# halajun/VDO_SLAM

Measured on AMD Instinct MI355X. Metric: frames/sec (per-frame hot path, KITTI-0000-shaped 1242x375) + ms/LM-iter (batch factor graph), higher is better.
Workload: dtype f64 (LM, RANSAC) / u8,i32,f32 (front-end, tracking)

## Files before the change

include/vdo_slam_hip.h:

```cpp
#ifndef VDO_SLAM_HIP_H_
#define VDO_SLAM_HIP_H_
#include <stdint.h>

#ifdef __cplusplus
extern "C" {
#endif

typedef enum vdo_status {
  VDO_OK = 0,
  VDO_ERR_INVALID = -1,
  VDO_ERR_NO_DEVICE = -2,
  VDO_ERR_OOM = -3,
  VDO_ERR_UNSUPPORTED = -4,
  VDO_ERR_INTERNAL = -5
} vdo_status;

int vdo_version(void);
const char* vdo_last_error(void);

typedef struct vdo_ctx vdo_ctx;
int vdo_ctx_create(int device, void* hip_stream, vdo_ctx** out);
int vdo_ctx_destroy(vdo_ctx* ctx);
int vdo_ctx_synchronize(vdo_ctx* ctx);
int vdo_ctx_stream(vdo_ctx* ctx, void** hip_stream_out);
// ... 31 lines not shown
  double* Hll_et;
  double* Hlp1_et;
  double* Hlp2_et;
  double* Hpp_ep;
  double chi2;
  double robust_chi2;
} vdo_ba_system;

typedef struct vdo_lm_options {
  int32_t max_iterations;
  double gain_threshold;
  int32_t verbose;
  int32_t solver;
  double pcg_tolerance;
  int32_t pcg_max_iterations;
} vdo_lm_options;

#define VDO_LM_MAX_TRACE 512
typedef struct vdo_lm_stats {
  int32_t iterations;
  int32_t total_trials;
  int32_t stop_reason;
  double initial_chi2, final_chi2, final_lambda;
  double chi2_trace[VDO_LM_MAX_TRACE];
  int32_t trials_trace[VDO_LM_MAX_TRACE];
  double ms_total, ms_linearize, ms_solve;
} vdo_lm_stats;

typedef struct vdo_ba vdo_ba;
int vdo_ba_create(vdo_ctx* ctx, const vdo_ba_graph* g, vdo_ba** out);
int vdo_ba_destroy(vdo_ba* ba);
int vdo_ba_linearize(vdo_ba* ba, int repeat, float* ms_sweep);
int vdo_ba_profile_linearize(vdo_ba* ba, int repeat, float ms[2], int64_t dims[8]);
int vdo_ba_profile_schur(vdo_ba* ba, int repeat, float* ms);
int vdo_ba_download_system(vdo_ba* ba, vdo_ba_system* out);
int vdo_ba_optimize(vdo_ba* ba, const vdo_lm_options* opt, vdo_lm_stats* stats);
int vdo_ba_get_estimates(vdo_ba* ba, double* pose_out , double* point_out );
int vdo_ba_set_estimates(vdo_ba* ba, const double* pose, const double* point);
typedef int (*vdo_allreduce_fn)(void* user, void* device_buf, int64_t count, int op);
int vdo_ba_set_allreduce(vdo_ba* ba, vdo_allreduce_fn fn, void* user, int shard_rank);
typedef struct vdo_rccl_comm vdo_rccl_comm;
int vdo_rccl_unique_id(char id_out[128]);
int vdo_rccl_comm_create(vdo_ctx* ctx, const char id[128], int n_ranks, int rank, vdo_rccl_comm** out);
int vdo_rccl_comm_destroy(vdo_rccl_comm* comm);
int vdo_rccl_comm_stats(const vdo_rccl_comm* comm, int64_t* calls, int64_t* bytes);
int vdo_rccl_allreduce(vdo_rccl_comm* comm, double* device_buf, int64_t count, int op );
int vdo_ba_set_rccl(vdo_ba* ba, vdo_rccl_comm* comm );
int vdo_ba_partition(const vdo_ba_graph* g, int world, int32_t* owner_of_point );
typedef struct vdo_ba_plan vdo_ba_plan;
int vdo_ba_plan_create(const vdo_ba_graph* g, vdo_ba_plan** out);
int vdo_ba_plan_array(const vdo_ba_plan* p, const char* name, const void** data, int64_t* count, int32_t* elem_bytes);
int vdo_ba_plan_destroy(vdo_ba_plan* p);

typedef struct vdo_flow2_problem {
  int32_t n;
  const double* obs;
  const double* flow;
  const double* depth;
  double K[4];
  double Twl[16];
  double T0[16];
  double info_flow;
  double info_prior;
  double huber_delta;
  double chi2_gate;
  int32_t max_iterations;
  int32_t ref_quirks;
} vdo_flow2_problem;

typedef struct vdo_flow2_result {
  double T[16];
  int32_t n_inliers;
  int32_t iterations, trials, stop_reason;
  double initial_chi2, final_chi2, final_lambda;
} vdo_flow2_result;

typedef struct vdo_flow2_batch vdo_flow2_batch;
int vdo_flow2_batch_create(vdo_ctx* ctx, int n_problems, const vdo_flow2_problem* probs, vdo_flow2_batch** out);
int vdo_flow2_batch_reserve(vdo_ctx* ctx, int n_problems, const int32_t* capacity, vdo_flow2_batch** out);
int vdo_flow2_batch_set(vdo_flow2_batch* batch, int k, const vdo_flow2_problem* problem);
int vdo_flow2_batch_set_T0(vdo_flow2_batch* batch, int k, const double T0[16]);
int vdo_flow2_batch_run(vdo_flow2_batch* batch);
int vdo_flow2_batch_fetch(vdo_flow2_batch* batch, vdo_flow2_result* results, double** flow_out, uint8_t** inlier_out);
int vdo_flow2_batch_destroy(vdo_flow2_batch* batch);
int vdo_flow2_optimize(vdo_ctx* ctx, const vdo_flow2_problem* p, vdo_flow2_result* result, double* flow_out, uint8_t* inlier_out);

typedef struct vdo_pose_problem {
  int32_t n;
  int32_t kind;
  const double* obs;
  const double* Xw;
  double K[4];
  double P[12];
  double T0[16];
  double huber_delta;
  double chi2_gate;
  int32_t max_iterations;
  int32_t pad;
} vdo_pose_problem;

typedef struct vdo_pose_batch vdo_pose_batch;
int vdo_pose_batch_create(vdo_ctx* ctx, int n_problems, const vdo_pose_problem* probs, vdo_pose_batch** out);
int vdo_pose_batch_run(vdo_pose_batch* batch);
int vdo_pose_batch_fetch(vdo_pose_batch* batch, vdo_flow2_result* results, uint8_t** inlier_out);
int vdo_pose_batch_destroy(vdo_pose_batch* batch);
int vdo_pose_optimize(vdo_ctx* ctx, const vdo_pose_problem* p, vdo_flow2_result* result, uint8_t* inlier_out);

typedef struct vdo_pnp_problem {
  int32_t n;
  const double* X;
  const double* uv;
  double K[4];
  int32_t max_iterations;
  double reproj_threshold;
  double confidence;
  int32_t refit;
} vdo_pnp_problem;
typedef struct vdo_pnp_result {
  double T[16];
  int32_t n_inliers;
  int32_t iterations_run;
  int32_t best_iteration;
} vdo_pnp_result;
int vdo_pnp_ransac_batch(vdo_ctx* ctx, int n_problems, const vdo_pnp_problem* probs, vdo_pnp_result* results, uint8_t** inlier_out);
int vdo_pnp_ransac_batch_overlap(vdo_ctx* ctx, int n_problems, const vdo_pnp_problem* probs, vdo_pnp_result* results, uint8_t** inlier_out,
                                 void (*host_work)(void*), void* host_arg);
int vdo_pnp_ransac_batch_gated(vdo_ctx* ctx, int n_problems, const vdo_pnp_problem* probs, vdo_pnp_result* results, uint8_t** inlier_out,
                               const int32_t* refit_above, void (*host_work)(void*), void* host_arg, void (*after_replay)(void*), void* after_arg);
int vdo_pnp_ransac(vdo_ctx* ctx, const vdo_pnp_problem* p, vdo_pnp_result* result, uint8_t* inlier_out);

typedef struct vdo_orb_params {
  int32_t n_features;
  float scale_factor;
  int32_t n_levels;
  int32_t ini_th;
  int32_t min_th;
} vdo_orb_params;

typedef struct vdo_keypoints {
  int32_t capacity, n;
  float *x, *y, *response, *angle, *size;
  int32_t* octave;
} vdo_keypoints;

typedef struct vdo_orb vdo_orb;
int vdo_orb_create(vdo_ctx* ctx, const vdo_orb_params* prm, int width, int height, vdo_orb** out);
int vdo_orb_destroy(vdo_orb* orb);
int vdo_orb_max_keypoints(const vdo_orb* orb, int* n);
int vdo_orb_last_keypoints(const vdo_orb* orb, int* n);
int vdo_orb_extract(vdo_orb* orb, const uint8_t* gray, int stride, int src_is_device, vdo_keypoints* out);
int vdo_orb_extract_begin(vdo_orb* orb, const uint8_t* gray, int stride, int src_is_device);
int vdo_orb_extract_end(vdo_orb* orb, vdo_keypoints* out);
int vdo_orb_descriptors(vdo_orb* orb, uint8_t* desc32, int capacity_rows);
int vdo_orb_extract_desc(vdo_orb* orb, const uint8_t* gray, int stride, int src_is_device, vdo_keypoints* out, uint8_t* desc32);
int vdo_orb_level_info(vdo_orb* orb, int level, int* w, int* h, int* n_features, int* n_candidates);
int vdo_orb_get_pyramid(vdo_orb* orb, int level, uint8_t* out_bordered );
int vdo_orb_get_blurred(vdo_orb* orb, int level, uint8_t* out );
int vdo_orb_get_candidates(vdo_orb* orb, int level, float* x, float* y, float* response, float* angle, int cap, int* n);
int vdo_orb_last_timing(vdo_orb* orb, double ms[2]);
int vdo_orb_tree_info(vdo_orb* orb, int level, int* on_device, int* status);
int vdo_orb_pyramid_launches(const vdo_orb* orb);


typedef struct vdo_match_set {
  int32_t n;
  const uint8_t* desc;
// ... 28 lines not shown
int vdo_frame_images_ingest_device(vdo_frame_images* f, const float* depth_dev, const float* flow_dev, const int32_t* mask_dev, float bf, float depth_map_factor,
                                   int convert_depth);
int vdo_frame_images_destroy(vdo_frame_images* f);
int vdo_frame_images_set_ctx(vdo_frame_images* f, vdo_ctx* ctx);
int vdo_frame_static_filter(vdo_frame_images* f, int n, const float* kx, const float* ky, float th_depth,
                            int32_t* keep_idx, float* corr_x, float* corr_y, float* flow_x, float* flow_y,
                            float* depth_out, int* n_out);
int vdo_frame_static_filter_sampled(vdo_frame_images* f, int n, const float* kx, const float* ky, float th_depth,
                                    int32_t* keep_idx, float* corr_x, float* corr_y, float* flow_x, float* flow_y,
                                    float* depth_out, int* n_out);
int vdo_sample_keypoints(int rows, int cols, uint64_t seed, int capacity, float* x_out, float* y_out, int* n_out);
int vdo_frame_object_sample(vdo_frame_images* f, float th_depth_obj, int step, int cap,
                            float* key_x, float* key_y, float* corr_x, float* corr_y,
                            float* flow_x, float* flow_y, float* depth_out, int32_t* label, int* n_out);
int vdo_frame_object_sample_on(vdo_ctx* on_ctx, vdo_frame_images* f, float th_depth_obj, int step, int cap,
                               float* key_x, float* key_y, float* corr_x, float* corr_y,
                               float* flow_x, float* flow_y, float* depth_out, int32_t* label, int* n_out);
int vdo_frame_filters(vdo_frame_images* f, int n, const float* kx, const float* ky, float th_depth, int sampled,
                      int32_t* keep_idx, float* s_corr_x, float* s_corr_y, float* s_flow_x, float* s_flow_y, float* s_depth, int* n_static,
                      float th_depth_obj, int step, int cap,
                      float* key_x, float* key_y, float* corr_x, float* corr_y, float* flow_x, float* flow_y, float* depth_out, int32_t* label, int* n_obj);
int vdo_frame_filters_on(vdo_ctx* on_ctx, vdo_frame_images* f, int n, const float* kx, const float* ky, float th_depth, int sampled,
                         int32_t* keep_idx, float* s_corr_x, float* s_corr_y, float* s_flow_x, float* s_flow_y, float* s_depth, int* n_static,
                         float th_depth_obj, int step, int cap,
                         float* key_x, float* key_y, float* corr_x, float* corr_y, float* flow_x, float* flow_y, float* depth_out, int32_t* label, int* n_obj);


int vdo_propagate_static(vdo_frame_images* f, int n, const float* kx, const float* ky, float* depth_out);
int vdo_propagate_object(vdo_frame_images* f, int n, const float* kx, const float* ky, float th_depth_obj,
                         float* depth_out, int32_t* label_out);
int vdo_get3d_world(vdo_ctx* ctx, int n, const float* kx, const float* ky, const float* depth,
                    const float K4[4], const float Twc[16], float* xyz_out);
int vdo_scene_flow(vdo_ctx* ctx, int n, const float* cur_x, const float* cur_y, const float* cur_d, const int32_t* cur_label, const float Tcw_cur[16],
                   const float* last_x, const float* last_y, const float* last_d, const int32_t* last_label, const float Tcw_last[16],
                   const float K4[4], float* flow3d_out, int32_t* obj_label_inout);
int vdo_renew_static(vdo_frame_images* f, int n_tm, const int32_t* tm_sta, const float* stat_x, const float* stat_y,
                     int n_orb, const float* orb_x, const float* orb_y, int max_num_sta,
                     float* key_x, float* key_y, float* corr_x, float* corr_y, float* flow_x, float* flow_y,
                     int32_t* inlier_id, float* depth_out, int* n_out);
int vdo_renew_static_world(vdo_frame_images* f, int n_tm, const int32_t* tm_sta, const float* stat_x, const float* stat_y,
                           int n_orb, const float* orb_x, const float* orb_y, int max_num_sta, const float K4[4], const float Twc[16],
                           float* key_x, float* key_y, float* corr_x, float* corr_y, float* flow_x, float* flow_y,
                           int32_t* inlier_id, float* depth_out, float* xyz_out, int* n_out);
int vdo_static_stage(vdo_frame_images* f, int n_orb, const float* orb_x, const float* orb_y, float th_depth,
                     int32_t* keep_idx, float* s_corr_x, float* s_corr_y, float* s_flow_x, float* s_flow_y, float* s_depth, int* n_static,
                     int n_tm, const int32_t* tm_sta, const float* stat_x, const float* stat_y, int max_num_sta, const float K4[4], const float Twc[16],
                     float* key_x, float* key_y, float* corr_x, float* corr_y, float* flow_x, float* flow_y,
                     int32_t* inlier_id, float* depth_out, float* xyz_out, int* n_out);
int vdo_mask_at(vdo_frame_images* f, int n, const float* cx, const float* cy, int32_t* label_out);
int vdo_mask_warp(vdo_frame_images* cur, vdo_frame_images* last, int32_t label);
int vdo_frame_images_download_mask(vdo_frame_images* f, int32_t* mask_out);
int vdo_frame_images_download_depth(vdo_frame_images* f, float* depth_out);
int vdo_frame_images_download_flow(vdo_frame_images* f, float* flow_out);


typedef struct vdo_dyn_obj_params {
  int32_t img_w, img_h;
  int32_t shrink_row, shrink_col;
  float sf_mg_thres, sf_ds_thres;
  float th_depth_obj;
  int32_t f_id;
} vdo_dyn_obj_params;
int vdo_dyn_obj_tracking(const vdo_dyn_obj_params* prm, int n, const int32_t* sem_label, int32_t* obj_label_inout,
                         const float* key_x, const float* key_y, const float* depth, const float* flow3d, const int32_t* last_sem_label,
                         int n_last_obj, const int32_t* last_sem_pos, const int32_t* last_mod_label, const uint8_t* last_obj_stat,
                         int32_t* max_id_inout, int32_t* obj_off, int32_t* obj_idx, int32_t* obj_sem, int32_t* obj_mod, int* n_obj_out);

int vdo_renew_object(vdo_frame_images* f, int n_obj, const int32_t* inl_off, const int32_t* inl_idx, const uint8_t* obj_stat,
                     const int32_t* sem_pos, const int32_t* mod_label,
                     const float* cur_x, const float* cur_y, const int32_t* cur_obj_label,
                     int n_tmp, const float* tmp_x, const float* tmp_y, const float* tmp_depth, const int32_t* tmp_label,
                     const float* tmp_flow_x, const float* tmp_flow_y, const float* tmp_corr_x, const float* tmp_corr_y,
                     int max_num_obj, int cap,
                     float* key_x, float* key_y, float* depth_out, int32_t* sem_out, float* flow_x, float* flow_y,
                     float* corr_x, float* corr_y, int32_t* dyn_inlier_id, int32_t* obj_label_out, int* n_out);
int vdo_renew_object_world(vdo_frame_images* f, int n_obj, const int32_t* inl_off, const int32_t* inl_idx, const uint8_t* obj_stat,
                           const int32_t* sem_pos, const int32_t* mod_label,
                           const float* cur_x, const float* cur_y, const int32_t* cur_obj_label,
                           int n_tmp, const float* tmp_x, const float* tmp_y, const float* tmp_depth, const int32_t* tmp_label,
                           const float* tmp_flow_x, const float* tmp_flow_y, const float* tmp_corr_x, const float* tmp_corr_y,
                           int max_num_obj, int cap, const float K4[4], const float Twc[16],
                           float* key_x, float* key_y, float* depth_out, int32_t* sem_out, float* flow_x, float* flow_y,
                           float* corr_x, float* corr_y, int32_t* dyn_inlier_id, int32_t* obj_label_out, float* xyz_out, int* n_out);

int vdo_update_mask(vdo_frame_images* cur, vdo_frame_images* last, int n, const int32_t* last_sem_label,
                    const float* last_corr_x, const float* last_corr_y, int* n_recovered);
int vdo_object_chain(vdo_frame_images* cur, vdo_frame_images* last, int n, const int32_t* last_sem_label, const float* last_corr_x, const float* last_corr_y,
                     float th_depth_obj, const float Tcw_cur[16], const float* last_x, const float* last_y, const float* last_d, const float Tcw_last[16],
                     const float K4[4], int* n_recovered, float* depth_out, int32_t* sem_out, float* flow3d_out, int32_t* obj_label_out);
int vdo_object_chain_begin(vdo_frame_images* cur, vdo_frame_images* last, int n, const int32_t* last_sem_label, const float* last_corr_x, const float* last_corr_y,
                           const float* last_x, const float* last_y, const float* last_d);
int vdo_object_chain_end(vdo_frame_images* cur, float th_depth_obj, const float Tcw_cur[16], const float Tcw_last[16], const float K4[4],
                         int* n_recovered, float* depth_out, int32_t* sem_out, float* flow3d_out, int32_t* obj_label_out);
int vdo_object_chain_prestage(vdo_ctx* ctx, int n, const int32_t* last_sem_label, const float* last_corr_x, const float* last_corr_y,
                              const float* last_x, const float* last_y, const float* last_d);

typedef struct vdo_tracks vdo_tracks;
int vdo_tracks_create(int with_object_label, vdo_tracks** out);
int vdo_tracks_destroy(vdo_tracks* t);
int vdo_tracks_add_frame(vdo_tracks* t, int n, const int32_t* asso , const int32_t* feat_label);
int vdo_tracks_size(vdo_tracks* t, int* n_tracks, int64_t* n_pairs);
int vdo_tracks_get(vdo_tracks* t, int32_t* track_off, int32_t* pair_frame, int32_t* pair_feat, int32_t* obj_id);
int vdo_tracks_get_since(vdo_tracks* t, int first_frame, int* n_tracks, int64_t* n_pairs, int32_t* track_off, int32_t* pair_frame, int32_t* pair_feat, int32_t* obj_id);

typedef struct vdo_ingest vdo_ingest;
typedef struct vdo_png_scanlines {
  const uint8_t* data;
  int64_t bytes;
  int32_t width, height, bit_depth, channels;
} vdo_png_scanlines;
enum { VDO_INGEST_MASK = 0, VDO_INGEST_FLO = 1, VDO_INGEST_DEPTH = 2, VDO_INGEST_COLOR = 3 };
int vdo_ingest_create(vdo_ctx* ctx, int width, int height, vdo_ingest** out);
int vdo_ingest_destroy(vdo_ingest* h);
int vdo_ingest_host_buffer(vdo_ingest* h, int which, int64_t bytes, void** ptr);
int vdo_ingest_device_outputs(vdo_ingest* h, uint8_t** gray, float** depth_raw, float** flow, int32_t** mask);
int vdo_ingest_frame(vdo_ingest* h, const char* mask_text, int64_t mask_bytes, const void* flo, int64_t flo_bytes, const vdo_png_scanlines* depth,
                     const vdo_png_scanlines* color, int rgb_order, uint8_t* gray, float* depth_raw, float* flow, int32_t* mask);
int vdo_ingest_last_timing(vdo_ingest* h, double ms[3]);

typedef struct vdo_stereo vdo_stereo;
typedef struct vdo_stereo_params {
  int32_t max_disparity;
  int32_t p1, p2;
  int32_t paths;
  int32_t uniqueness;
  int32_t lr_max_diff;
  int32_t subpixel;
} vdo_stereo_params;
int vdo_stereo_create(vdo_ctx* ctx, int width, int height, const vdo_stereo_params* params, vdo_stereo** out);
int vdo_stereo_destroy(vdo_stereo* h);
int vdo_stereo_compute(vdo_stereo* h, const uint8_t* left, int64_t left_stride, const uint8_t* right, int64_t right_stride, int src_is_device,
                       float* disparity256, int out_is_device, int32_t* n_valid);
int vdo_stereo_set_output_scale(vdo_stereo* h, float scale);
int vdo_stereo_get_census(vdo_stereo* h, int which, uint64_t* out);
int vdo_stereo_get_cost(vdo_stereo* h, uint8_t* out);
int vdo_stereo_get_aggregated(vdo_stereo* h, uint16_t* out);
int vdo_stereo_last_timing(vdo_stereo* h, double ms[2]);
int vdo_stereo_device_images(vdo_stereo* h, uint8_t** left, uint8_t** right, float** disparity256);
int vdo_stereo_stage_frame(vdo_stereo* h, const float* flow, const int32_t* mask, float** flow_dev, int32_t** mask_dev);

typedef struct vdo_optflow vdo_optflow;
typedef struct vdo_optflow_params {
  int32_t levels;
  int32_t radius;
  int32_t window;
  int32_t median;
  int32_t fb_max_diff;
  int32_t subpixel;
} vdo_optflow_params;
int vdo_optflow_create(vdo_ctx* ctx, int width, int height, const vdo_optflow_params* params, vdo_optflow** out);
int vdo_optflow_destroy(vdo_optflow* h);
int vdo_optflow_compute(vdo_optflow* h, const uint8_t* im0, int64_t stride0, const uint8_t* im1, int64_t stride1, int src_is_device, float* flow,
                        uint8_t* valid, int out_is_device, int32_t* n_valid);
int vdo_optflow_level_size(vdo_optflow* h, int level, int* width, int* height);
int vdo_optflow_get_pyramid(vdo_optflow* h, int which, int level, uint8_t* out);
int vdo_optflow_get_census(vdo_optflow* h, int which, int level, uint64_t* out);
int vdo_optflow_get_level_flow(vdo_optflow* h, int dir, int level, int32_t* out);
int vdo_optflow_last_timing(vdo_optflow* h, double ms[2]);
int vdo_optflow_device_images(vdo_optflow* h, uint8_t** im0, uint8_t** im1, float** flow, uint8_t** valid);
int vdo_optflow_stage_mask(vdo_optflow* h, const int32_t* mask, int32_t** mask_dev);

typedef struct vdo_labels vdo_labels;
typedef struct vdo_labels_params {
  int32_t connectivity;
  int32_t max_disp_diff;
  int32_t min_area;
// ... 207 lines not shown
```

vdo_slam_amd/csrc/capi_ctx.hip:

```cpp
#include <cstdlib>
#include <cstdarg>
#include <cstdio>

#include "../../include/vdo_slam_hip.h"
#include "ctx.hpp"

namespace {
thread_local char g_err[512] = "";
}

namespace vdo {
int set_error(int code, const char* fmt, ...) {
  va_list ap;
  va_start(ap, fmt);
  std::vsnprintf(g_err, sizeof(g_err), fmt, ap);
  va_end(ap);
  return code;
}
int ctx_bind(vdo_ctx* ctx) {
  if (!ctx) return set_error(VDO_ERR_INVALID, "null context");
  hipError_t e = hipSetDevice(ctx->device);
  if (e != hipSuccess) return set_error(VDO_ERR_NO_DEVICE, "hipSetDevice(%d): %s", ctx->device, hipGetErrorString(e));
  return VDO_OK;
}
}

extern "C" int vdo_version(void) { return 1; }
extern "C" const char* vdo_last_error(void) { return g_err; }

extern "C" int vdo_ctx_create(int device, void* hip_stream, vdo_ctx** out) {
  if (!out) return vdo::set_error(VDO_ERR_INVALID, "vdo_ctx_create: null out");
  int n = 0;
  hipError_t e = hipGetDeviceCount(&n);
  if (e != hipSuccess || n <= 0)
    return vdo::set_error(VDO_ERR_NO_DEVICE, "no HIP device available (%s); libvdo_hip has no CPU fallback",
                          e == hipSuccess ? "device count 0" : hipGetErrorString(e));
  if (device < 0 || device >= n) return vdo::set_error(VDO_ERR_INVALID, "device %d out of range [0,%d)", device, n);
  vdo_ctx* c = new vdo_ctx();
  c->device = device;
  if (hipSetDevice(device) != hipSuccess) { delete c; return vdo::set_error(VDO_ERR_NO_DEVICE, "hipSetDevice failed"); }
  if (hip_stream) { c->stream = (hipStream_t)hip_stream; c->owns_stream = false; }
  else {
    if (hipStreamCreateWithFlags(&c->stream, hipStreamNonBlocking) != hipSuccess) { delete c; return vdo::set_error(VDO_ERR_NO_DEVICE, "hipStreamCreate failed"); }
    c->owns_stream = true;
  }
  *out = c;
  return VDO_OK;
}

extern "C" int vdo_ctx_destroy(vdo_ctx* ctx) {
  if (!ctx) return VDO_OK;
  hipSetDevice(ctx->device);
  if (ctx->chain_open) {
    hipStreamSynchronize(ctx->stream);
    ctx->chain_open_free(ctx->chain_open);
  }
  if (ctx->d_arena) hipFree(ctx->d_arena);
  if (ctx->h_arena) hipHostFree(ctx->h_arena);
  if (ctx->ba_slab) hipFree(ctx->ba_slab);
  if (ctx->ba_hscal) hipHostFree(ctx->ba_hscal);
  if (ctx->ba_side) hipStreamDestroy(ctx->ba_side);
  for (hipEvent_t e : ctx->ba_ev) if (e) hipEventDestroy(e);
  if (ctx->d_stage) hipFree(ctx->d_stage);
  if (ctx->h_stage) hipHostFree(ctx->h_stage);
  if (ctx->owns_stream && ctx->stream) hipStreamDestroy(ctx->stream);
  delete ctx;
  return VDO_OK;
}

extern "C" int vdo_ctx_synchronize(vdo_ctx* ctx) {
  int rc = vdo::ctx_bind(ctx);
  if (rc != VDO_OK) return rc;
  hipError_t e = hipStreamSynchronize(ctx->stream);
  if (e != hipSuccess) return vdo::set_error(VDO_ERR_NO_DEVICE, "hipStreamSynchronize: %s", hipGetErrorString(e));
  return VDO_OK;
}

extern "C" int vdo_ctx_stream(vdo_ctx* ctx, void** hip_stream_out) {
  if (!ctx || !hip_stream_out) return vdo::set_error(VDO_ERR_INVALID, "vdo_ctx_stream: null argument");
  *hip_stream_out = (void*)ctx->stream;
  return VDO_OK;
}

extern "C" int vdo_ctx_create_cu_mask(int device, int cu_first, int cu_count, int invert, vdo_ctx** out) {
  if (!out || cu_first < 0 || cu_count <= 0) return vdo::set_error(VDO_ERR_INVALID, "vdo_ctx_create_cu_mask: bad argument");
  int n = 0;
  hipError_t e = hipGetDeviceCount(&n);
  if (e != hipSuccess || n <= 0)
    return vdo::set_error(VDO_ERR_NO_DEVICE, "no HIP device available (%s); libvdo_hip has no CPU fallback", e == hipSuccess ? "device count 0" : hipGetErrorString(e));
  if (device < 0 || device >= n) return vdo::set_error(VDO_ERR_INVALID, "device %d out of range [0,%d)", device, n);
  if (hipSetDevice(device) != hipSuccess) return vdo::set_error(VDO_ERR_NO_DEVICE, "hipSetDevice failed");
  hipDeviceProp_t prop;
  if (hipGetDeviceProperties(&prop, device) != hipSuccess) return vdo::set_error(VDO_ERR_NO_DEVICE, "hipGetDeviceProperties failed");
  const int ncu = prop.multiProcessorCount;
  if (cu_first + cu_count > ncu) return vdo::set_error(VDO_ERR_INVALID, "CU range [%d,%d) exceeds the %d CUs of the device", cu_first, cu_first + cu_count, ncu);
  const int words = (ncu + 31) / 32;
  uint32_t mask[32] = {0};
  for (int c = 0; c < ncu; ++c) {
    const bool in = c >= cu_first && c < cu_first + cu_count;
    if (in != (invert != 0)) mask[c / 32] |= 1u << (c % 32);
  }
  vdo_ctx* c = new vdo_ctx();
  c->device = device;
  if (hipExtStreamCreateWithCUMask(&c->stream, (uint32_t)words, mask) != hipSuccess) { delete c; return vdo::set_error(VDO_ERR_NO_DEVICE, "hipExtStreamCreateWithCUMask failed"); }
  c->owns_stream = true;
  *out = c;
  return VDO_OK;
}
```

vdo_slam_amd/csrc/ctx.hpp:

```cpp
#pragma once
#include <hip/hip_runtime.h>

#include <cstddef>
#include <cstdint>

struct vdo_ctx {
  int device = 0;
  hipStream_t stream = nullptr;
  bool owns_stream = false;
  char* d_arena = nullptr; size_t d_cap = 0;
  char* h_arena = nullptr; size_t h_cap = 0;
  char* h_arena_dev = nullptr;
  void* chain_open = nullptr; void (*chain_open_free)(void*) = nullptr; bool arena_held = false;
  char* d_stage = nullptr; char* h_stage = nullptr; size_t stage_cap = 0;
  int stage_n = -1, stage_L = 0;
  int32_t stage_uni[64]; int32_t stage_off[65];
  char* ba_slab = nullptr; size_t ba_slab_cap = 0, ba_slab_used = 0; bool ba_pool_busy = false;
  double* ba_hscal = nullptr; double* ba_hscal_dev = nullptr;
  hipStream_t ba_side = nullptr; hipEvent_t ba_ev[4] = {nullptr, nullptr, nullptr, nullptr};
};

namespace vdo {
int set_error(int code, const char* fmt, ...) __attribute__((format(printf, 2, 3)));
int ctx_bind(vdo_ctx* ctx);
}
```

vdo_slam_amd/csrc/flow2.hip:

```cpp
#include <algorithm>
#include <cmath>
#include <cstdlib>
#include <cstring>
#include <type_traits>
#include <vector>

#include "../../include/vdo_slam_hip.h"
#include "ctx.hpp"
#include "lm_dev.hpp"

namespace vdo {

struct Flow2Dev {
  int n, max_iterations, ref_quirks, pad;
  int64_t off;
  int64_t out_off, out_total;
  double K[4], Twl[16], T0[16];
  double info_flow, info_prior, huber_delta, huber_dsqr, chi2_gate;
};

struct Flow2Arrays {
  const double* in;
  double* om;
  double *Xw, *f0, *f1, *err, *B2a, *B2b, *hla, *hlb, *bla, *blb, *xl;
  char* out;
  int n_problems;
  struct Flow2Comm* comm;
  unsigned int tag_base;
  int max_cluster;
  int force_general;
};

constexpr int F2_CLUSTER = 8;
static_assert(F2_THREADS >= 32 * F2_CLUSTER, "cluster exchange: one thread per (workgroup, value)");
struct Flow2Slot { unsigned int lo, tag_lo, hi, tag_hi; };
struct Flow2Comm {
  Flow2Slot slot[2][F2_CLUSTER][32];
};
typedef unsigned int f2_u32x4 __attribute__((ext_vector_type(4)));
#ifndef F2_XSCOPE
#define F2_XSCOPE 2
#endif
#if F2_XSCOPE == 3
#define F2_SC "sc0 sc1"
#elif F2_XSCOPE == 2
#define F2_SC "sc1"
#else
#define F2_SC "sc0"
#endif
__device__ __forceinline__ void f2_slot_store(Flow2Slot* p, const f2_u32x4 w) { asm volatile("global_store_dwordx4 %0, %1, off " F2_SC :: "v"(p), "v"(w) : "memory"); }
__device__ __forceinline__ f2_u32x4 f2_slot_load(const Flow2Slot* p) {
  f2_u32x4 w;
  asm volatile("global_load_dwordx4 %0, %1, off " F2_SC "\n\ts_waitcnt vmcnt(0)" : "=v"(w) : "v"(p) : "memory");
  return w;
}

struct F2Pre { double B[12], b0, b1, d0, d1, d2, p2; int i; };

struct F2Lin { double B[12], h, b0, b1; };

struct F2RegStore {
  static constexpr bool kReg = true;
  const int i, tid;
  const bool active;
  double* const s_h;
  double o0 = 0, o1 = 0, m0 = 0, m1 = 0, xw[3] = {0, 0, 0};
  double fc0 = 0, fc1 = 0, ft0 = 0, ft1 = 0, xl0 = 0, xl1 = 0, er0 = 0, er1 = 0;
  F2Lin cur{}, trial{};
  double hpc = 0, hpt = 0;
  template <class F> __device__ __forceinline__ void for_each(F&& f) { if (active) f(i); }
  __device__ __forceinline__ void set_point(int, double a0, double a1, double b0, double b1, const double (&x)[3]) {
    o0 = a0; o1 = a1; m0 = b0; m1 = b1; xw[0] = x[0]; xw[1] = x[1]; xw[2] = x[2]; fc0 = b0; fc1 = b1; xl0 = 0; xl1 = 0;
  }
  __device__ __forceinline__ void point(int, double& a0, double& a1, double& b0, double& b1, double (&x)[3]) const {
    a0 = o0; a1 = o1; b0 = m0; b1 = m1; x[0] = xw[0]; x[1] = xw[1]; x[2] = xw[2];
  }
  __device__ __forceinline__ void flow_cur(int, double& f0, double& f1) const { f0 = fc0; f1 = fc1; }
  __device__ __forceinline__ void set_flow_try(int, double f0, double f1) { ft0 = f0; ft1 = f1; }
  __device__ __forceinline__ void get_xl(int, double& x0, double& x1) const { x0 = xl0; x1 = xl1; }
  __device__ __forceinline__ void set_xl(int, double x0, double x1) { xl0 = x0; xl1 = x1; }
  __device__ __forceinline__ void get_err(int, double& e0, double& e1) const { e0 = er0; e1 = er1; }
  __device__ __forceinline__ void set_err(int, double e0, double e1) { er0 = e0; er1 = e1; }
  __device__ __forceinline__ void lin_cur(int, F2Lin& L) const { L = cur; }
  template <bool TRIAL> __device__ __forceinline__ void set_lin(int, const F2Lin& L) {
    if constexpr (TRIAL) trial = L; else cur = L;
    s_h[tid] = L.h;
  }
  __device__ __forceinline__ double h_prev(int, double) const { return hpc; }
  template <bool TRIAL> __device__ __forceinline__ void after_exchange(double hb) {
    const double h = tid > 0 ? s_h[tid - 1] : hb;
    if constexpr (TRIAL) hpt = h; else hpc = h;
// ... 427 lines not shown
          if (tid < 27) s_Hc[tid] = s_red[tid];
          if (tid == 32) s_T = s_Ttry;
        } else {
          lambda *= ni; ni *= 2; built = false;
        }
        __syncthreads();
        F2_TICK(3);
        ++qmax; ++total_trials;
      } while (rho < 0 && qmax < 10);
      int result;
      if (qmax == 10 || rho == 0) result = 1;
      else {
        if ((iniChi - currentChi) * 1e3 < iniChi) nBad++; else nBad = 0;
        result = nBad >= 3 ? 1 : 0;
      }
      ok = (result == 0);
      if (!ok) stop_reason = 1;
      if (chi2_check < last_err_chi && it > 0) { ok = false; stop_reason = 2; }
      chi2_check = last_err_chi;
    }
    double cnt[1] = {0.0};
    const float gate = (float)P.chi2_gate;
    S.for_each([&](const int i) {
      double e0, e1, f0, f1;
      S.get_err(i, e0, e1);
      S.flow_cur(i, f0, f1);
      const float chi2 = (float)(e0 * (P.info_flow * e0) + e1 * (P.info_flow * e1));
      const bool outl = chi2 > gate;
      inlier_out[i] = outl ? 0 : 1;
      cnt[0] += outl ? 0.0 : 1.0;
      flow_out[2 * i] = f0;
      flow_out[2 * i + 1] = f1;
    });
    block_reduce<1>(cnt, s_scr, s_red);
    { double d_ = 0, e_ = 0; F2_CLUSTER_SUM(1, d_, e_); }
    if (tid == 0 && wg == 0) {
      se3_to_matrix(s_T, res->T);
      res->n_inliers = (int)(s_red[0] + 0.5);
      res->iterations = it; res->trials = total_trials; res->stop_reason = stop_reason;
      res->initial_chi2 = initial_chi2; res->final_chi2 = last_err_chi; res->final_lambda = lambda;
#ifdef F2_PROFILE
      for (int k = 0; k < 14; ++k) res->T[k] = (double)s_prof[k];
#endif
    }
#ifdef F2_PROFILE
    __syncthreads();
    if (tid == 0 && wg < 2) res->T[14 + wg] = (double)(__builtin_amdgcn_s_getreg((4 - 1) << 11 | 0 << 6 | 20) & 0xf) + 100.0 * blockIdx.x;
#endif
  };

  const bool REG = chunk <= F2_THREADS && !A.force_general;
  if (REG) {
    __shared__ double s_h[F2_THREADS];
    F2RegStore S{first, tid, first < c_hi, s_h};
    lm_body(S);
  } else {
    double* const om = A.om + 4 * off;
    F2MemStore S{N, first, c_lo, c_hi, om, om + 2 * (size_t)N, A.Xw + 3 * off, A.f0 + 2 * off, A.f1 + 2 * off, A.err + 2 * off, A.xl + 2 * off,
                 A.B2a + 12 * off, A.B2b + 12 * off, A.hla + off, A.hlb + off, A.bla + 2 * off, A.blb + 2 * off};
    lm_body(S);
  }
}

}

using namespace vdo;

struct vdo_flow2_batch {
  vdo_ctx* ctx = nullptr;
  int n_problems = 0;
  int64_t total = 0;
  std::vector<void*> allocs;
  Flow2Dev* d_probs = nullptr;
  Flow2Arrays A{};
  std::vector<int64_t> offs;
  std::vector<int> ns;
  char* h_pin = nullptr;
  double* h_up = nullptr;
  std::vector<Flow2Dev> hp;
  std::vector<int> caps;
  bool probs_dirty = false;
  unsigned run_seq = 0;
  const Flow2Dev* d_probs_run = nullptr;
};

extern "C" int vdo_flow2_batch_destroy(vdo_flow2_batch* b) {
  if (!b) return VDO_OK;
  if (b->ctx) { ctx_bind(b->ctx); hipStreamSynchronize(b->ctx->stream); }
  for (void* p : b->allocs) hipFree(p);
  if (b->h_pin) hipHostFree(b->h_pin);
  if (b->h_up) hipHostFree(b->h_up);
  delete b;
  return VDO_OK;
}

static void fill_descriptor(Flow2Dev& d, const vdo_flow2_problem& p) {
  d.max_iterations = p.max_iterations; d.ref_quirks = p.ref_quirks;
  std::memcpy(d.K, p.K, sizeof(d.K)); std::memcpy(d.Twl, p.Twl, sizeof(d.Twl)); std::memcpy(d.T0, p.T0, sizeof(d.T0));
  d.info_flow = p.info_flow; d.info_prior = p.info_prior; d.huber_delta = p.huber_delta;
  d.huber_dsqr = (double)(float)(p.huber_delta * p.huber_delta);
  d.chi2_gate = p.chi2_gate;
}

static void pack_planes(double* st, const vdo_flow2_problem& p) {
  const size_t n = (size_t)p.n;
  double *po = st, *pm = st + 2 * n;
  for (size_t i = 0; i < n; ++i) { po[i] = p.obs[2 * i]; po[n + i] = p.obs[2 * i + 1]; pm[i] = p.flow[2 * i]; pm[n + i] = p.flow[2 * i + 1]; }
  std::memcpy(st + 4 * n, p.depth, sizeof(double) * n);
}

extern "C" int vdo_flow2_batch_create(vdo_ctx* ctx, int n_problems, const vdo_flow2_problem* probs, vdo_flow2_batch** out) {
  if (!ctx || !probs || !out || n_problems <= 0) return set_error(VDO_ERR_INVALID, "vdo_flow2_batch_create: bad argument");
  int rc = ctx_bind(ctx);
  if (rc != VDO_OK) return rc;
  vdo_flow2_batch* b = new vdo_flow2_batch();
  b->ctx = ctx; b->n_problems = n_problems;
  std::vector<Flow2Dev> hp(n_problems);
  int64_t total = 0;
  for (int k = 0; k < n_problems; ++k) {
    const vdo_flow2_problem& p = probs[k];
    if (p.n < 0 || (p.n > 0 && (!p.obs || !p.flow || !p.depth))) { delete b; return set_error(VDO_ERR_INVALID, "flow2 problem %d: null input", k); }
    Flow2Dev& d = hp[k];
    fill_descriptor(d, p);
    d.n = p.n; d.pad = 0; d.off = total; d.out_off = total;
    b->offs.push_back(total); b->ns.push_back(p.n);
    total += p.n;
  }
  for (Flow2Dev& d : hp) d.out_total = total;
  b->total = total;
  hipStream_t s = ctx->stream;
  auto dev = [&](size_t bytes) -> void* {
    void* p = nullptr;
    if (bytes == 0) bytes = 8;
    if (hipMalloc(&p, bytes) != hipSuccess) return nullptr;
    b->allocs.push_back(p);
    return p;
  };
  const size_t T = (size_t)total, NP = (size_t)n_problems;
  std::vector<double> in(5 * T);
  for (int k = 0; k < n_problems; ++k) if (probs[k].n) pack_planes(in.data() + 5 * b->offs[k], probs[k]);
  double* d_in = (double*)dev(40 * T);
  b->d_probs = (Flow2Dev*)dev(sizeof(Flow2Dev) * NP);
  Flow2Arrays& A = b->A;
  A.in = d_in;
  A.om = (double*)dev(32 * T);
  A.Xw = (double*)dev(24 * T); A.f0 = (double*)dev(16 * T); A.f1 = (double*)dev(16 * T);
  A.err = (double*)dev(16 * T); A.B2a = (double*)dev(96 * T); A.B2b = (double*)dev(96 * T);
  A.hla = (double*)dev(8 * T); A.hlb = (double*)dev(8 * T); A.bla = (double*)dev(16 * T); A.blb = (double*)dev(16 * T);
  A.xl = (double*)dev(16 * T);
  A.n_problems = n_problems;
  A.comm = (Flow2Comm*)dev(sizeof(Flow2Comm) * NP);
  if (A.comm) hipMemsetAsync(A.comm, 0, sizeof(Flow2Comm) * NP, s);
  for (void* p : b->allocs) if (!p) { vdo_flow2_batch_destroy(b); return set_error(VDO_ERR_OOM, "hipMalloc failed"); }
  if (!d_in) { vdo_flow2_batch_destroy(b); return set_error(VDO_ERR_OOM, "hipMalloc failed"); }
  hipMemcpyAsync(d_in, in.data(), 40 * T, hipMemcpyHostToDevice, s);
  hipMemcpyAsync(b->d_probs, hp.data(), sizeof(Flow2Dev) * NP, hipMemcpyHostToDevice, s);
  if (hipHostMalloc((void**)&b->h_pin, sizeof(vdo_flow2_result) * NP + 16 * T + T + 64, hipHostMallocMapped) != hipSuccess) { b->h_pin = nullptr; vdo_flow2_batch_destroy(b); return set_error(VDO_ERR_OOM, "hipHostMalloc failed"); }
  {
    void* dp = nullptr;
    if (hipHostGetDevicePointer(&dp, b->h_pin, 0) != hipSuccess || !dp) { vdo_flow2_batch_destroy(b); return set_error(VDO_ERR_NO_DEVICE, "hipHostGetDevicePointer failed"); }
    A.out = (char*)dp;
  }
  if (hipStreamSynchronize(s) != hipSuccess) { vdo_flow2_batch_destroy(b); return set_error(VDO_ERR_NO_DEVICE, "flow2 upload failed"); }
  b->hp = hp; b->caps = b->ns;
  *out = b;
  return VDO_OK;
}

extern "C" int vdo_flow2_batch_reserve(vdo_ctx* ctx, int n_problems, const int32_t* capacity, vdo_flow2_batch** out) {
  if (!ctx || !capacity || !out || n_problems <= 0) return set_error(VDO_ERR_INVALID, "vdo_flow2_batch_reserve: bad argument");
  int64_t tot = 0;
  for (int k = 0; k < n_problems; ++k) { if (capacity[k] < 0) return set_error(VDO_ERR_INVALID, "negative capacity"); tot += capacity[k]; }
  std::vector<double> zeros(2 * (size_t)std::max<int64_t>(1, *std::max_element(capacity, capacity + n_problems)), 0.0);
  std::vector<vdo_flow2_problem> dummy(n_problems);
  for (int k = 0; k < n_problems; ++k) {
    std::memset(&dummy[k], 0, sizeof(vdo_flow2_problem));
    dummy[k].n = capacity[k]; dummy[k].obs = zeros.data(); dummy[k].flow = zeros.data(); dummy[k].depth = zeros.data();
  }
  int rc = vdo_flow2_batch_create(ctx, n_problems, dummy.data(), out);
  if (rc != VDO_OK) return rc;
  vdo_flow2_batch* b = *out;
  if (hipHostMalloc((void**)&b->h_up, sizeof(double) * 5 * (size_t)std::max<int64_t>(tot, 1) + sizeof(Flow2Dev) * (size_t)n_problems, hipHostMallocMapped) != hipSuccess) { b->h_up = nullptr; vdo_flow2_batch_destroy(b); return set_error(VDO_ERR_OOM, "hipHostMalloc failed"); }
  void* dp = nullptr;
  if (hipHostGetDevicePointer(&dp, b->h_up, 0) != hipSuccess || !dp) { vdo_flow2_batch_destroy(b); return set_error(VDO_ERR_NO_DEVICE, "hipHostGetDevicePointer failed"); }
  b->A.in = (const double*)dp;
  b->d_probs_run = (const Flow2Dev*)((const double*)dp + 5 * (size_t)std::max<int64_t>(tot, 1));
  for (int k = 0; k < n_problems; ++k) { b->hp[k].n = 0; b->ns[k] = 0; }
  std::memcpy(b->h_up + 5 * (size_t)std::max<int64_t>(tot, 1), b->hp.data(), sizeof(Flow2Dev) * (size_t)n_problems);
  if (hipStreamSynchronize(ctx->stream) != hipSuccess) { vdo_flow2_batch_destroy(b); return set_error(VDO_ERR_NO_DEVICE, "flow2 reserve failed"); }
  return VDO_OK;
}

extern "C" int vdo_flow2_batch_set(vdo_flow2_batch* b, int k, const vdo_flow2_problem* p) {
  if (!b || k < 0 || k >= b->n_problems || !b->h_up) return set_error(VDO_ERR_INVALID, "vdo_flow2_batch_set: bad argument / batch not created by vdo_flow2_batch_reserve");
  int rc = ctx_bind(b->ctx);
  if (rc != VDO_OK) return rc;
  Flow2Dev& d = b->hp[k];
  const int n = p ? p->n : 0;
  if (n < 0 || n > b->caps[k] || (n > 0 && (!p->obs || !p->flow || !p->depth))) return set_error(VDO_ERR_INVALID, "vdo_flow2_batch_set: %d points do not fit slot %d (capacity %d)", n, k, b->caps[k]);
  if (n) {
    pack_planes(b->h_up + 5 * b->offs[k], *p);
    fill_descriptor(d, *p);
  }
  d.n = n; b->ns[k] = n;
  b->probs_dirty = true;
  return VDO_OK;
}

extern "C" int vdo_flow2_batch_set_T0(vdo_flow2_batch* b, int k, const double T0[16]) {
  if (!b || k < 0 || k >= b->n_problems || !b->h_up || !T0) return set_error(VDO_ERR_INVALID, "vdo_flow2_batch_set_T0: bad argument / batch not created by vdo_flow2_batch_reserve");
  std::memcpy(b->hp[k].T0, T0, sizeof(b->hp[k].T0));
  b->probs_dirty = true;
  return VDO_OK;
}

extern "C" int vdo_flow2_batch_run(vdo_flow2_batch* b) {
  if (!b) return set_error(VDO_ERR_INVALID, "null handle");
  int rc = ctx_bind(b->ctx);
  if (rc != VDO_OK) return rc;
  if (b->probs_dirty) {
    int64_t used = 0;
    for (int k = 0; k < b->n_problems; ++k) { b->hp[k].out_off = used; used += b->hp[k].n; }
    for (int k = 0; k < b->n_problems; ++k) b->hp[k].out_total = used;
    std::memcpy(b->h_up + 5 * (size_t)std::max<int64_t>(b->total, 1), b->hp.data(), sizeof(Flow2Dev) * (size_t)b->n_problems);
    b->probs_dirty = false;
  }
  b->A.tag_base = (++b->run_seq) << 16;
  {
    int budget = 256;
    if (const char* e = std::getenv("VDO_LM_CLUSTER_BUDGET")) budget = std::max(1, std::atoi(e));
    int mc = F2_CLUSTER;
    for (; mc > 1; mc >>= 1) {
      int64_t wgs = 0;
      for (int k = 0; k < b->n_problems; ++k) if (b->ns[k] >= 3) wgs += std::min(mc, std::max(1, (b->ns[k] + F2_THREADS - 1) / F2_THREADS));
      if (wgs <= budget) break;
    }
    b->A.max_cluster = mc;
  }
  { const char* e = std::getenv("VDO_LM_GENERAL"); b->A.force_general = (e && std::atoi(e) != 0) ? 1 : 0; }
  hipLaunchKernelGGL(k_flow2_lm, dim3(((b->n_problems + 7) / 8) * 8 * F2_CLUSTER), dim3(F2_THREADS), 0, b->ctx->stream, b->d_probs_run ? b->d_probs_run : (const Flow2Dev*)b->d_probs, b->A);
  hipError_t e = hipGetLastError();
  if (e != hipSuccess) return set_error(VDO_ERR_NO_DEVICE, "k_flow2_lm launch: %s", hipGetErrorString(e));
  return VDO_OK;
}

extern "C" int vdo_flow2_batch_fetch(vdo_flow2_batch* b, vdo_flow2_result* results, double** flow_out, uint8_t** inlier_out) {
  if (!b || !results) return set_error(VDO_ERR_INVALID, "null argument");
  int rc = ctx_bind(b->ctx);
  if (rc != VDO_OK) return rc;
  const size_t NP = (size_t)b->n_problems;
  size_t used = 0;
  for (int k = 0; k < b->n_problems; ++k) used += (size_t)b->ns[k];
  hipError_t e = hipStreamSynchronize(b->ctx->stream);
  if (e != hipSuccess) return set_error(VDO_ERR_NO_DEVICE, "flow2 fetch: %s", hipGetErrorString(e));
  const vdo_flow2_result* pr = (const vdo_flow2_result*)b->h_pin;
  const double* pf = (const double*)(b->h_pin + sizeof(vdo_flow2_result) * NP);
  const uint8_t* pi = (const uint8_t*)(pf + 2 * used);
  std::memcpy(results, pr, sizeof(vdo_flow2_result) * NP);
  for (size_t k = 0; k < NP; ++k) if (pr[k].iterations < 0) return set_error(VDO_ERR_NO_DEVICE, "k_flow2_lm: the workgroup cluster of problem %d lost its barrier", (int)k);
  size_t o = 0;
  for (int k = 0; k < b->n_problems; ++k) {
    const size_t n = (size_t)b->ns[k];
    if (n && flow_out && flow_out[k]) std::memcpy(flow_out[k], pf + 2 * o, sizeof(double) * 2 * n);
    if (n && inlier_out && inlier_out[k]) std::memcpy(inlier_out[k], pi + o, n);
    o += n;
  }
  return VDO_OK;
}

extern "C" int vdo_flow2_optimize(vdo_ctx* ctx, const vdo_flow2_problem* p, vdo_flow2_result* result, double* flow_out, uint8_t* inlier_out) {
  vdo_flow2_batch* b = nullptr;
  int rc = vdo_flow2_batch_create(ctx, 1, p, &b);
  if (rc != VDO_OK) return rc;
  rc = vdo_flow2_batch_run(b);
  if (rc == VDO_OK) rc = vdo_flow2_batch_fetch(b, result, &flow_out, &inlier_out);
  vdo_flow2_batch_destroy(b);
  return rc;
}
```

vdo_slam_amd/csrc/tracking_logic.hip:

```cpp
#include <algorithm>
#include <chrono>
#include <cmath>
#include <cstring>
#include <vector>

#include "../../include/vdo_slam_hip.h"
#include "ctx.hpp"
#include "frame_images.hpp"
#include "near_flags.hpp"
#include "arena.hpp"
#include "tracking_shared.hpp"

namespace vdo {

__global__ void k_renew_obj_pred(int n, const float* __restrict__ px, const float* __restrict__ py, const int32_t* __restrict__ mask,
                                 const float* __restrict__ depth, const float* __restrict__ flow, int w, int h,
                                 int32_t* __restrict__ ok, int32_t* __restrict__ sem, float* __restrict__ dout, float* __restrict__ fx, float* __restrict__ fy) {
  const int i = blockIdx.x * blockDim.x + threadIdx.x;
  if (i >= n) return;
  const int x = (int)px[i], y = (int)py[i];
  int good = 0, sl = 0;
  float d = 0, fxe = 0, fye = 0;
  if (!(x >= w || y >= h || x <= 0 || y <= 0)) {
    const size_t o = (size_t)y * w + x;
    sl = mask[o]; d = depth[o];
    if (sl != 0 && d < 25 && d > 0) {
      fxe = flow[2 * o]; fye = flow[2 * o + 1];
      if (x + fxe < w && y + fye < h && x + fxe > 0 && y + fye > 0) good = 1;
    }
  }
  ok[i] = good; sem[i] = sl; dout[i] = d; fx[i] = fxe; fy[i] = fye;
}

__global__ void k_renew_obj_all(int n, const float* __restrict__ px, const float* __restrict__ py, const int32_t* __restrict__ mask,
                                const float* __restrict__ depth, const float* __restrict__ flow, int w, int h,
                                int32_t* __restrict__ ok, int32_t* __restrict__ sem, float* __restrict__ dout, float* __restrict__ fx, float* __restrict__ fy,
                                Cam cam, float* __restrict__ xyz_c,
                                int n_tmp, const float* __restrict__ qx, const float* __restrict__ qy, const float* __restrict__ qd, float* __restrict__ xyz_t,
                                int32_t* __restrict__ used) {
  const int i = blockIdx.x * blockDim.x + threadIdx.x;
  if (i < n) {
    const int x = (int)px[i], y = (int)py[i];
    int good = 0, sl = 0;
    float d = 0, fxe = 0, fye = 0;
    if (!(x >= w || y >= h || x <= 0 || y <= 0)) {
      const size_t o = (size_t)y * w + x;
      sl = mask[o]; d = depth[o];
      if (sl != 0 && d < 25 && d > 0) {
        fxe = flow[2 * o]; fye = flow[2 * o + 1];
        if (x + fxe < w && y + fye < h && x + fxe > 0 && y + fye > 0) good = 1;
      }
    }
    ok[i] = good; sem[i] = sl; dout[i] = d; fx[i] = fxe; fy[i] = fye;
    float o3[3];
    backproject(cam, (float)x, (float)y, d, o3);
    xyz_c[3 * i] = o3[0]; xyz_c[3 * i + 1] = o3[1]; xyz_c[3 * i + 2] = o3[2];
  }
  if (i < n_tmp) {
    used[i] = 0;
    float o3[3];
    backproject(cam, qx[i], qy[i], qd[i], o3);
    xyz_t[3 * i] = o3[0]; xyz_t[3 * i + 1] = o3[1]; xyz_t[3 * i + 2] = o3[2];
  }
}

constexpr int kVoteBins = 1024;

__global__ __launch_bounds__(256) void k_label_vote(int n, const float* __restrict__ cx, const float* __restrict__ cy,
                                                    const int32_t* __restrict__ mask, int w, int h, int32_t* __restrict__ flag) {
  __shared__ int hist[kVoteBins];
  __shared__ int s_valid, s_bad;
  for (int i = threadIdx.x; i < kVoteBins; i += 256) hist[i] = 0;
  if (threadIdx.x == 0) { s_valid = 0; s_bad = 0; }
  __syncthreads();
  for (int i = threadIdx.x; i < n; i += 256) {
    const int u = (int)cx[i], v = (int)cy[i];
    if (u < w && u > 0 && v < h && v > 0) {
      const int l = mask[(size_t)v * w + u];
      if (l < 0 || l >= kVoteBins) atomicOr(&s_bad, 1);
      else { atomicAdd(&hist[l], 1); atomicAdd(&s_valid, 1); }
    }
  }
  __syncthreads();
  __shared__ int s_cnt[256], s_lab[256];
  {
    int best = threadIdx.x * 4, cnt = hist[best];
    for (int l = best + 1; l < threadIdx.x * 4 + 4; ++l) if (hist[l] > cnt) { cnt = hist[l]; best = l; }
    s_cnt[threadIdx.x] = cnt; s_lab[threadIdx.x] = best;
  }
  __syncthreads();
  for (int step = 128; step > 0; step >>= 1) {
    if (threadIdx.x < step) {
      const int c2 = s_cnt[threadIdx.x + step], l2 = s_lab[threadIdx.x + step];
      if (c2 > s_cnt[threadIdx.x] || (c2 == s_cnt[threadIdx.x] && l2 < s_lab[threadIdx.x])) { s_cnt[threadIdx.x] = c2; s_lab[threadIdx.x] = l2; }
    }
    __syncthreads();
  }
  if (threadIdx.x == 0) {
    flag[0] = (s_valid >= 100 && s_lab[0] == 0 && !s_bad) ? 1 : 0;
    flag[1] = s_bad;
  }
}

__global__ void k_mask_warp_if(const int32_t* __restrict__ flag, const int32_t* __restrict__ mask_last, const float* __restrict__ flow_last,
                               int w, int h, int32_t lab, int32_t* __restrict__ mask_cur) {
  if (!flag[0]) return;
  const int k = blockIdx.x * blockDim.x + threadIdx.x, j = blockIdx.y;
  if (k >= w) return;
  const size_t o = (size_t)j * w + k;
  if (mask_last[o] != lab) return;
  const int fx = (int)flow_last[2 * o], fy = (int)flow_last[2 * o + 1];
  if (k + fx < w && k + fx > 0 && j + fy < h && j + fy > 0) mask_cur[(size_t)(j + fy) * w + (k + fx)] = lab;
}

struct LabelSlots { int n; int32_t lab[64]; };

__global__ __launch_bounds__(256) void k_warp_candidates(const int32_t* __restrict__ mask_last, const float* __restrict__ flow_last, int w, int h, LabelSlots T,
                                                         unsigned long long* __restrict__ cand) {
  const int k = blockIdx.x * blockDim.x + threadIdx.x, j = blockIdx.y;
  if (k >= w) return;
  const size_t o = (size_t)j * w + k;
  const int32_t lab = mask_last[o];
  int slot = -1;
  for (int s = 0; s < T.n; ++s) if (T.lab[s] == lab) slot = s;
  if (slot < 0) return;
  const int fx = (int)flow_last[2 * o], fy = (int)flow_last[2 * o + 1];
  if (k + fx < w && k + fx > 0 && j + fy < h && j + fy > 0) atomicOr(&cand[(size_t)(j + fy) * w + (k + fx)], 1ull << slot);
}

struct VoteLds { int hist[kVoteBins]; int valid, bad; int cnt[256], lab[256]; int verdict; };
__device__ __forceinline__ int vote_label(VoteLds& L, const LabelSlots& T, int s, unsigned long long rec, const int32_t* __restrict__ off, const float* __restrict__ cx,
                                          const float* __restrict__ cy, const int32_t* __restrict__ mask, const unsigned long long* __restrict__ cand, int w, int h,
                                          int32_t* __restrict__ flag) {
  for (int i = threadIdx.x; i < kVoteBins; i += 256) L.hist[i] = 0;
  if (threadIdx.x == 0) { L.valid = 0; L.bad = 0; }
  __syncthreads();
  const int lo = off[s], hi = off[s + 1];
  for (int base = lo + (int)(threadIdx.x & ~63u); base < hi; base += 4 * 256) {
    float px[4], py[4];
#pragma unroll
    for (int k = 0; k < 4; ++k) { const int i = min(base + k * 256 + (int)(threadIdx.x & 63u), hi - 1); px[k] = cx[i]; py[k] = cy[i]; }
    int ml[4]; unsigned long long mc[4]; bool in[4];
#pragma unroll
    for (int k = 0; k < 4; ++k) {
      const int i = base + k * 256 + (int)(threadIdx.x & 63u);
      const int u = (int)px[k], v = (int)py[k];
// ... 138 lines not shown
  }
  std::sort(v.begin(), v.end());
  int best = 0, cnt = -1;
  for (size_t a = 0; a < v.size();) {
    size_t b = a;
    while (b < v.size() && v[b] == v[a]) ++b;
    if ((int)(b - a) > cnt) { cnt = (int)(b - a); best = v[a]; }
    a = b;
  }
  return best;
}

}

using namespace vdo;

extern "C" int vdo_dyn_obj_tracking(const vdo_dyn_obj_params* prm, int n, const int32_t* sem_label, int32_t* obj_label_inout,
                                    const float* key_x, const float* key_y, const float* depth, const float* flow3d, const int32_t* last_sem_label,
                                    int n_last_obj, const int32_t* last_sem_pos, const int32_t* last_mod_label, const uint8_t* last_obj_stat,
                                    int32_t* max_id_inout, int32_t* obj_off, int32_t* obj_idx, int32_t* obj_sem, int32_t* obj_mod, int* n_obj_out) {
  if (!prm || !n_obj_out || !max_id_inout || n < 0 || (n > 0 && (!sem_label || !obj_label_inout || !key_x || !key_y || !depth || !flow3d || !last_sem_label)))
    return set_error(VDO_ERR_INVALID, "vdo_dyn_obj_tracking: bad argument");
  std::vector<int32_t> uni, slot;
  label_slots(n, sem_label, uni, slot);
  const int L = (int)uni.size();
  std::vector<int> cnt(L, 0);
  std::vector<float> border(L, 0.f);
  for (int i = 0; i < n; ++i) {
    if (obj_label_inout[i] == -1) continue;
    const int s = slot[i];
    ++cnt[s];
    const float u = key_x[i], v = key_y[i];
    if (v < prm->shrink_row || v > (prm->img_h - prm->shrink_row) || u < prm->shrink_col || u > (prm->img_w - prm->shrink_col)) border[s] += 1.f;
  }
  std::vector<int> state(L, 0);
  for (int s = 0; s < L; ++s) if (border[s] / (float)cnt[s] > 0.5f) state[s] = 1;
  std::vector<float> dsum(L, 0.f), slow(L, 0.f);
  for (int i = 0; i < n; ++i) {
    if (obj_label_inout[i] == -1) continue;
    const int s = slot[i];
    if (state[s] == 1) { obj_label_inout[i] = -1; continue; }
    dsum[s] = dsum[s] + depth[i];
    const float fx = flow3d[3 * i], fz = flow3d[3 * i + 2];
    if (std::sqrt(fx * fx + fz * fz) < prm->sf_mg_thres) slow[s] = slow[s] + 1.f;
  }
  for (int s = 0; s < L; ++s) {
    if (state[s]) continue;
    if (slow[s] / (float)cnt[s] > prm->sf_ds_thres) state[s] = 2;
    else if (dsum[s] / (float)cnt[s] > prm->th_depth_obj || cnt[s] < 150) state[s] = 3;
  }
  std::vector<int> acc_of(L, -1);
  int n_acc = 0;
  obj_off[0] = 0;
  for (int s = 0; s < L; ++s) if (state[s] == 0) { acc_of[s] = n_acc; obj_off[n_acc + 1] = obj_off[n_acc] + cnt[s]; obj_sem[n_acc] = uni[s]; ++n_acc; }
  std::vector<int> cur(n_acc + 1);
  for (int a = 0; a <= n_acc; ++a) cur[a] = obj_off[a];
  for (int i = 0; i < n; ++i) {
    if (obj_label_inout[i] == -1) continue;
    const int s = slot[i];
    if (state[s] == 2) obj_label_inout[i] = 0;
    else if (state[s] == 3) obj_label_inout[i] = -1;
    else if (state[s] == 0) obj_idx[cur[acc_of[s]]++] = i;
  }
  int max_id = *max_id_inout;
  if (prm->f_id == 1) max_id = 1;
  std::vector<int32_t> votes;
  for (int a = 0; a < n_acc; ++a) {
    votes.clear();
    for (int q = obj_off[a]; q < obj_off[a + 1]; ++q) votes.push_back(last_sem_label[obj_idx[q]]);
    const int new_lab = majority(votes);
    int lab = -1;
    if (max_id != 1)
      for (int k = 0; k < n_last_obj; ++k)
        if (last_sem_pos[k] == new_lab && last_obj_stat[k]) { lab = last_mod_label[k]; break; }
    if (lab == -1) { lab = max_id; max_id = max_id + 1; }
    for (int q = obj_off[a]; q < obj_off[a + 1]; ++q) obj_label_inout[obj_idx[q]] = lab;
    obj_mod[a] = lab;
  }
  *max_id_inout = max_id;
  *n_obj_out = n_acc;
  return VDO_OK;
}

extern "C" int vdo_renew_object_world(vdo_frame_images* f, int n_obj, const int32_t* inl_off, const int32_t* inl_idx, const uint8_t* obj_stat,
                                      const int32_t* sem_pos, const int32_t* mod_label,
                                      const float* cur_x, const float* cur_y, const int32_t* cur_obj_label,
                                      int n_tmp, const float* tmp_x, const float* tmp_y, const float* tmp_depth, const int32_t* tmp_label,
                                      const float* tmp_flow_x, const float* tmp_flow_y, const float* tmp_corr_x, const float* tmp_corr_y,
                                      int max_num_obj, int cap, const float K4[4], const float Twc[16],
                                      float* key_x, float* key_y, float* depth_out, int32_t* sem_out, float* flow_x, float* flow_y,
                                      float* corr_x, float* corr_y, int32_t* dyn_inlier_id, int32_t* obj_label_out, float* xyz_out, int* n_out) {
  if (!f || !n_out || n_obj < 0 || n_tmp < 0 || cap < 0 || (xyz_out && (!K4 || !Twc))) return set_error(VDO_ERR_INVALID, "vdo_renew_object: bad argument");
  int rc = ctx_bind(f->ctx);
  if (rc != VDO_OK) return rc;
  Arena S(f->ctx);
  if (!S.reserve(Arena::bytes_for(24 * ((size_t)(n_obj ? inl_off[n_obj] : 0) + (size_t)n_tmp + 64)))) return set_error(VDO_ERR_OOM, "scratch arena: allocation failed");
  static thread_local std::vector<float> cx, cy, dd, fx, fy, xyz_c, xyz_t;
  static thread_local std::vector<int32_t> cid, cobj, ok, sem, used;
  cx.clear(); cy.clear(); cid.clear(); cobj.clear();
  for (int i = 0; i < n_obj; ++i) {
    if (!obj_stat[i]) continue;
    for (int q = inl_off[i]; q < inl_off[i + 1]; ++q) { const int id = inl_idx[q]; cx.push_back(cur_x[id]); cy.push_back(cur_y[id]); cid.push_back(id); cobj.push_back(i); }
  }
  const int nc = (int)cx.size();
  ok.resize(nc); sem.resize(nc); dd.resize(nc); fx.resize(nc); fy.resize(nc);
  used.assign(n_tmp, 0);
  xyz_c.resize(xyz_out ? 3 * (size_t)nc : 0); xyz_t.resize(xyz_out ? 3 * (size_t)n_tmp : 0);
  if (nc || (n_tmp && xyz_out)) {
    float *dx = S.up(cx.data(), nc), *dy = S.up(cy.data(), nc);
    float *dqx = S.up(tmp_x, n_tmp), *dqy = S.up(tmp_y, n_tmp), *dqd = S.up(xyz_out ? tmp_depth : nullptr, xyz_out ? n_tmp : 0);
    int32_t *dok = S.up<int32_t>(nullptr, nc), *dsem = S.up<int32_t>(nullptr, nc);
    float *ddd = S.up<float>(nullptr, nc), *dfx = S.up<float>(nullptr, nc), *dfy = S.up<float>(nullptr, nc);
    int32_t* dused = S.up<int32_t>(nullptr, n_tmp);
    float *dxc = S.up<float>(nullptr, xyz_out ? 3 * (size_t)nc : 0), *dxt = S.up<float>(nullptr, xyz_out ? 3 * (size_t)n_tmp : 0);
    if (!dxt || !dxc || !dused || !dfy) return set_error(VDO_ERR_OOM, "scratch arena: allocation failed");
    hipStream_t st = S.stream();
    const Cam cam = xyz_out ? make_cam_Twc(K4, Twc) : Cam{};
    if (xyz_out) {
      const int nmax = std::max(nc, n_tmp);
      hipLaunchKernelGGL(k_renew_obj_all, dim3((nmax + 255) / 256), dim3(256), 0, st, nc, (const float*)dx, (const float*)dy, (const int32_t*)f->d_mask,
                         (const float*)f->d_depth, (const float*)f->d_flow, f->w, f->h, dok, dsem, ddd, dfx, dfy, cam, dxc,
                         n_tmp, (const float*)dqx, (const float*)dqy, (const float*)dqd, dxt, dused);
      if (nc && n_tmp) launch_near_flags_sel(st, n_tmp, dqx, dqy, nc, dx, dy, dok, 1, dused, false);
    } else if (nc) {
      hipLaunchKernelGGL(k_renew_obj_pred, dim3((nc + 255) / 256), dim3(256), 0, st, nc, (const float*)dx, (const float*)dy, (const int32_t*)f->d_mask,
                         (const float*)f->d_depth, (const float*)f->d_flow, f->w, f->h, dok, dsem, ddd, dfx, dfy);
      if (n_tmp) launch_near_flags_sel(st, n_tmp, dqx, dqy, nc, dx, dy, dok, 1, dused);
    }
    S.down(ok.data(), dok, nc); S.down(sem.data(), dsem, nc); S.down(dd.data(), ddd, nc); S.down(fx.data(), dfx, nc); S.down(fy.data(), dfy, nc);
    if (nc && n_tmp) S.down(used.data(), dused, n_tmp);
    if (xyz_out) { S.down(xyz_c.data(), dxc, 3 * (size_t)nc); S.down(xyz_t.data(), dxt, 3 * (size_t)n_tmp); }
    rc = S.finish("vdo_renew_object");
    if (rc != VDO_OK) return rc;
  }
  int m = 0;
  auto push = [&](float x, float y, float d, int sl, float flx, float fly, float crx, float cry, int inl, int ol, const float* p3) -> bool {
    if (m >= cap) return false;
    key_x[m] = x; key_y[m] = y; depth_out[m] = d; sem_out[m] = sl; flow_x[m] = flx; flow_y[m] = fly; corr_x[m] = crx; corr_y[m] = cry;
    dyn_inlier_id[m] = inl; obj_label_out[m] = ol;
    if (xyz_out) { xyz_out[3 * m] = p3[0]; xyz_out[3 * m + 1] = p3[1]; xyz_out[3 * m + 2] = p3[2]; }
    ++m;
    return true;
  };
  std::vector<int> fea_count(n_obj, -1);
  for (int i = 0; i < n_obj; ++i) if (obj_stat[i]) fea_count[i] = 0;
  for (int k = 0; k < nc; ++k) {
    if (!ok[k]) continue;
    const int x = (int)cx[k], y = (int)cy[k];
    if (!push((float)x, (float)y, dd[k], sem[k], fx[k], fy[k], x + fx[k], y + fy[k], cid[k], cur_obj_label[cid[k]], xyz_c.data() + 3 * (size_t)k)) return set_error(VDO_ERR_INVALID, "vdo_renew_object: output capacity %d too small", cap);
    ++fea_count[cobj[k]];
  }
  for (int i = 0; i < n_obj; ++i) {
    if (!obj_stat[i]) continue;
    int tot = fea_count[i];
    for (int start = 0; start < 15 && tot < max_num_obj; ++start) {
      for (int j = start; j < n_tmp; j += 15) {
        if (tmp_label[j] != sem_pos[i] || used[j]) continue;
        if (!push(tmp_x[j], tmp_y[j], tmp_depth[j], tmp_label[j], tmp_flow_x[j], tmp_flow_y[j], tmp_corr_x[j], tmp_corr_y[j], -1, mod_label[i], xyz_t.data() + 3 * (size_t)j))
          return set_error(VDO_ERR_INVALID, "vdo_renew_object: output capacity %d too small", cap);
        if (++tot >= max_num_obj) break;
      }
    }
  }
  std::vector<int32_t> uni, slot;
  label_slots(n_tmp, tmp_label, uni, slot);
  std::vector<char> known(uni.size(), 0);
  for (int i = 0; i < n_obj; ++i) {
    if (!obj_stat[i]) continue;
    auto it = std::lower_bound(uni.begin(), uni.end(), sem_pos[i]);
    if (it != uni.end() && *it == sem_pos[i]) known[it - uni.begin()] = 1;
  }
  for (size_t s = 0; s < uni.size(); ++s) {
    if (known[s]) continue;
    for (int j = 0; j < n_tmp; ++j)
      if (slot[j] == (int)s && !push(tmp_x[j], tmp_y[j], tmp_depth[j], tmp_label[j], tmp_flow_x[j], tmp_flow_y[j], tmp_corr_x[j], tmp_corr_y[j], -1, -2, xyz_t.data() + 3 * (size_t)j))
        return set_error(VDO_ERR_INVALID, "vdo_renew_object: output capacity %d too small", cap);
  }
  *n_out = m;
  return VDO_OK;
}

extern "C" int vdo_renew_object(vdo_frame_images* f, int n_obj, const int32_t* inl_off, const int32_t* inl_idx, const uint8_t* obj_stat,
                                const int32_t* sem_pos, const int32_t* mod_label,
                                const float* cur_x, const float* cur_y, const int32_t* cur_obj_label,
                                int n_tmp, const float* tmp_x, const float* tmp_y, const float* tmp_depth, const int32_t* tmp_label,
                                const float* tmp_flow_x, const float* tmp_flow_y, const float* tmp_corr_x, const float* tmp_corr_y,
                                int max_num_obj, int cap,
                                float* key_x, float* key_y, float* depth_out, int32_t* sem_out, float* flow_x, float* flow_y,
                                float* corr_x, float* corr_y, int32_t* dyn_inlier_id, int32_t* obj_label_out, int* n_out) {
  return vdo_renew_object_world(f, n_obj, inl_off, inl_idx, obj_stat, sem_pos, mod_label, cur_x, cur_y, cur_obj_label, n_tmp, tmp_x, tmp_y, tmp_depth, tmp_label,
                                tmp_flow_x, tmp_flow_y, tmp_corr_x, tmp_corr_y, max_num_obj, cap, nullptr, nullptr,
                                key_x, key_y, depth_out, sem_out, flow_x, flow_y, corr_x, corr_y, dyn_inlier_id, obj_label_out, nullptr, n_out);
}

extern "C" int vdo_update_mask(vdo_frame_images* cur, vdo_frame_images* last, int n, const int32_t* last_sem_label,
                               const float* last_corr_x, const float* last_corr_y, int* n_recovered) {
  if (!cur || !last || cur->w != last->w || cur->h != last->h || n < 0) return set_error(VDO_ERR_INVALID, "vdo_update_mask: bad argument");
  if (n_recovered) *n_recovered = 0;
  if (n == 0) return VDO_OK;
  int rc = ctx_bind(cur->ctx);
  if (rc != VDO_OK) return rc;
  Arena S(cur->ctx);
  if (!S.reserve(Arena::bytes_for(4 * (size_t)n + 512))) return set_error(VDO_ERR_OOM, "scratch arena: allocation failed");
  std::vector<int32_t> uni, slot;
  label_slots(n, last_sem_label, uni, slot);
  const int L = (int)uni.size();
  std::vector<int> off(L + 1, 0);
  for (int i = 0; i < n; ++i) off[slot[i] + 1]++;
  for (int s = 0; s < L; ++s) off[s + 1] += off[s];
  std::vector<float> gx(n), gy(n);
  {
    std::vector<int> c(off.begin(), off.end() - 1);
    for (int i = 0; i < n; ++i) { const int p = c[slot[i]]++; gx[p] = last_corr_x[i]; gy[p] = last_corr_y[i]; }
  }
  float *dx = S.up(gx.data(), n), *dy = S.up(gy.data(), n);
  std::vector<int32_t> off32(off.begin(), off.end());
  int32_t* doff = S.up(off32.data(), off32.size());
  int32_t* dflag = S.up<int32_t>(nullptr, 2 * (size_t)L);
  unsigned long long* drec = S.up<unsigned long long>(nullptr, 1);
  if (!dflag || !doff || !drec) return set_error(VDO_ERR_OOM, "hipMalloc failed");
  launch_update_mask(cur, last, uni, off, dx, dy, doff, dflag, drec, S.stream());
  std::vector<int32_t> flag(2 * (size_t)L);
  S.down(flag.data(), dflag, flag.size());
  rc = S.finish("vdo_update_mask");
  if (rc != VDO_OK) return rc;
  int rec = 0;
  for (int s = 0; s < L; ++s) {
    if (flag[2 * s + 1]) return set_error(VDO_ERR_UNSUPPORTED, "vdo_update_mask: mask label outside [0,%d)", kVoteBins);
    rec += flag[2 * s];
  }
  if (n_recovered) *n_recovered = rec;
  return VDO_OK;
}

static __global__ void k_gather_scene_flow(int n, const float* __restrict__ kx, const float* __restrict__ ky, const float* __restrict__ depth, const int32_t* __restrict__ mask,
                                           int w, int h, float th, float* __restrict__ dout, int32_t* __restrict__ lout, Cam cc,
                                           const float* __restrict__ lx, const float* __restrict__ ly, const float* __restrict__ ld, const int32_t* __restrict__ ll, Cam lc,
                                           float* __restrict__ flow3d, int32_t* __restrict__ objlab, const int32_t* __restrict__ olab_init,
                                           const int32_t* __restrict__ flag_in, int32_t* __restrict__ flag_out, int nflag) {
  const int i = blockIdx.x * blockDim.x + threadIdx.x;
  if (i < nflag) flag_out[i] = flag_in[i];
  if (i >= n) return;
  const float xf = kx[i], yf = ky[i];
  const int u = (int)xf, v = (int)yf;
  float o = 0.1f; int l = 0;
  {
    const bool inside = u < (w - 1) && u > 0 && v < (h - 1) && v > 0;
    const size_t q = inside ? (size_t)v * w + u : 0;
    const float d = depth[q];
    const int ml = mask[q];
    if (inside && d < th && d > 0) { o = d; l = ml; }
  }
  dout[i] = o; lout[i] = l;
  if (l <= 0 || ll[i] <= 0) { objlab[i] = -1; flow3d[3 * i] = 0; flow3d[3 * i + 1] = 0; flow3d[3 * i + 2] = 0; return; }
  float p[3], c[3];
  backproject(lc, lx[i], ly[i], ld[i], p);
  backproject(cc, xf, yf, o, c);
  flow3d[3 * i] = c[0] - p[0]; flow3d[3 * i + 1] = c[1] - p[1]; flow3d[3 * i + 2] = c[2] - p[2];
  objlab[i] = olab_init ? olab_init[i] : -2;
}

namespace {
struct ChainLayout { size_t gx, gy, cx, cy, lx, ly, ld, ll, off, total; };
ChainLayout chain_layout(int n) {
  auto al = [](size_t v) { return (v + 255) & ~size_t(255); };
  ChainLayout q{};
  size_t o = 0;
  const size_t b = al(4 * (size_t)n);
  q.gx = o; o += b; q.gy = o; o += b; q.cx = o; o += b; q.cy = o; o += b; q.lx = o; o += b; q.ly = o; o += b; q.ld = o; o += b; q.ll = o; o += b;
  q.off = o; o += al(4 * 65);
  q.total = o;
  return q;
}
int group_by_label(int n, const int32_t* lab, const float* px, const float* py, std::vector<int32_t>& uni, std::vector<int>& off, float* gx, float* gy) {
  static thread_local std::vector<int32_t> slot;
// ... 266 lines not shown
```

vdo_slam_amd/host/FramePipeline.cc:

```cpp
#include "FramePipeline.h"

#include "Optimizer.h"
#include "frame_math.h"

#include <algorithm>
#include <cmath>
#include <cstdio>
#include <cstdlib>
#include <cstring>
#include <thread>
#include <stdexcept>

namespace VDO_SLAM {

using namespace frame_math;

namespace {
struct SecTimer {
  double* ms; std::chrono::steady_clock::time_point t = std::chrono::steady_clock::now();
  void reset() { t = std::chrono::steady_clock::now(); }
  void tick(int slot) { const auto n = std::chrono::steady_clock::now(); ms[slot] += std::chrono::duration<double, std::milli>(n - t).count(); t = n; }
};
int await_tag(const std::atomic<int>& a, int tag) {
  for (int v;; std::this_thread::yield()) if ((v = a.load(std::memory_order_acquire)) == tag || v == -tag) return v;
}
}

class FramePipeline::Worker {
 public:
  Worker() : th_([this] { loop(); }) {}
  ~Worker() { state_.store(3, std::memory_order_release); th_.join(); }
  void run(std::function<int()> job) { job_ = std::move(job); state_.store(1, std::memory_order_release); }
  int wait() {
    if (!busy()) return 0;
    while (state_.load(std::memory_order_acquire) != 2) std::this_thread::yield();
    state_.store(0, std::memory_order_relaxed);
    return rc_;
  }
  bool busy() const { const int s = state_.load(std::memory_order_acquire); return s == 1 || s == 2; }

 private:
  void loop() {
    unsigned idle = 0;
    for (;;) {
      const int s = state_.load(std::memory_order_acquire);
      if (s == 3) return;
      if (s == 1) { rc_ = job_(); state_.store(2, std::memory_order_release); idle = 0; continue; }
      if (++idle < 200000u) continue;
      if (idle < 400000u) std::this_thread::yield(); else std::this_thread::sleep_for(std::chrono::microseconds(200));
    }
  }
  std::function<int()> job_;
  int rc_ = 0;
  std::atomic<int> state_{0};
  std::thread th_;
};

struct FramePipeline::StepState {
  FramePipeline& P;
  const uint8_t* d_gray; const float *d_depth_raw, *d_flow; const int32_t* d_mask;
  vdo_flow2_batch *cam, *obj; int n_cam_pts, n_obj_problems;
  vdo_frame_images *cur, *last;
  ObjSet& tmp;
  vdo_keypoints kp;
  const int tag;
  FrameCounts fc{};
  bool orb_pending = false, tail_via_orb = false, k10_via_orb = false, k9_via_orb = false, fin_async = false, late_upload = false, up_async = false, static_async = false,
       tail_async = false, tail_on_orb = false;
  bool orb_started = false;
  bool chain_open = false;
  int n_s = 0, n_o = 0, n_new_s = 0, n_tmp = 0, n_objects = 0;
  float Tcw[16];
  StaSet nsta; ObjSet nobj;
  std::vector<int32_t> sta_asso;
  SecTimer t;
  StepState(FramePipeline& p, const uint8_t* g, const float* d, const float* f, const int32_t* m, vdo_flow2_batch* c, vdo_flow2_batch* o, int nc, int no)
      : P(p), d_gray(g), d_depth_raw(d), d_flow(f), d_mask(m), cam(c), obj(o), n_cam_pts(nc), n_obj_problems(no), cur(p.img_[p.cur_]), last(p.img_[p.cur_ ^ 1]),
        tmp(p.tmpb_[p.cur_]), kp{(int32_t)p.kx_.size(), 0, p.kx_.data(), p.ky_.data(), p.kr_.data(), p.ka_.data(), p.ks_.data(), p.ko_.data()}, tag(p.f_id_ + 1), t{p.ms_} {}
  ~StepState() {
    if (P.worker_) P.worker_->wait();
    if (chain_open) vdo_object_chain_end(cur, 0.f, kI4, kI4, P.p_.K4, nullptr, nullptr, nullptr, nullptr, nullptr);
    for (std::atomic<int>* a : {&P.objects_done_, &P.mask_final_}) { const int v = a->load(); if (v != tag && v != -tag) a->store(-tag); }
    if (orb_started) P.worker_orb_->wait();
    if (P.worker_) P.worker_->wait();
  }
};

#define VDO_TRY(call) do { if ((call) != VDO_OK) { std::fprintf(stderr, "FramePipeline: %s\n", vdo_last_error()); return -1; } } while (0)

FramePipeline::Switches FramePipeline::ReadSwitches() {
  auto on = [](const char* name) { return std::getenv(name) != nullptr; };
  Switches w;
  w.events = on("VDO_PIPE_EVENTS"); w.trace_slow = on("VDO_PIPE_TRACE_SLOW"); w.trace_obj = on("VDO_PIPE_TRACE_OBJ"); w.trace_batch = on("VDO_BATCH_TRACE");
  w.sync_upload = on("VDO_PIPE_SYNC_UPLOAD"); w.async_upload = !on("VDO_PIPE_NO_ASYNC_UPLOAD"); w.chain_split = !on("VDO_PIPE_NO_CHAIN_SPLIT");
  w.fused_static = !on("VDO_PIPE_NO_FUSED_STATIC"); w.k9_in_static = on("VDO_PIPE_K9_IN_STATIC"); w.mm_overlap = !on("VDO_PIPE_NO_MM_OVERLAP"); w.cam_ahead = !on("VDO_PIPE_NO_CAM_AHEAD");
  return w;
}

FramePipeline::FramePipeline(vdo_ctx* ctx, vdo_ctx* ctx_lm, const PipelineParams& p, vdo_ctx* ctx_obj, vdo_ctx* ctx_worker, vdo_ctx* ctx_orb)
    : ctx_(ctx), ctx_lm_(ctx_lm), ctx_obj_(ctx_obj ? ctx_obj : ctx_lm), ctx_w_(ctx_worker ? ctx_worker : ctx), p_(p) {
  vdo_orb_params op{p.n_features, p.scale_factor, p.n_levels, p.ini_th, p.min_th};
  if (vdo_orb_create(ctx_orb ? ctx_orb : ctx, &op, p.width, p.height, &orb_) != VDO_OK) return;
  for (int k = 0; k < 2; ++k) if (vdo_frame_images_create(ctx, p.width, p.height, &img_[k]) != VDO_OK) return;
  if (vdo_tracks_create(0, &tr_sta_) != VDO_OK || vdo_tracks_create(1, &tr_dyn_) != VDO_OK) return;
  int orb_cap = 0;
  if (vdo_orb_max_keypoints(orb_, &orb_cap) != VDO_OK) return;
  const int capk = std::max(orb_cap, 3008);
  kx_.resize(capk); ky_.resize(capk); kr_.resize(capk); ka_.resize(capk); ks_.resize(capk); ko_.resize(capk);
  for (int i = 0; i < 16; ++i) Tcw_last_[i] = vel_[i] = kI4[i];
  if (p.build_lm) {
    const int32_t ccap = std::max({p.max_track_bg + 8, p.n_features + 256, orb_cap});
    if (vdo_flow2_batch_reserve(ctx_lm, 1, &ccap, &lm_cam_) != VDO_OK) return;
    std::vector<int32_t> ocap(obj_slots_, obj_cap_);
    if (vdo_flow2_batch_reserve(ctx_obj_, obj_slots_, ocap.data(), &lm_obj_) != VDO_OK) return;
  }
  store_.sta.reserve((size_t)1 << 20); store_.dyn.reserve((size_t)1 << 22);
  if (ctx_worker) worker_.reset(new Worker());
  if (ctx_worker && ctx_orb) worker_orb_.reset(new Worker());
  ctx_orb_ = ctx_orb;
  orb_split_ = ctx_orb != nullptr;
  ok_ = true;
}

FramePipeline::~FramePipeline() {
  if (worker_) { worker_->wait(); worker_.reset(); }
  if (worker_orb_) { worker_orb_->wait(); worker_orb_.reset(); }
  if (orb_) vdo_orb_destroy(orb_);
  for (int k = 0; k < 2; ++k) if (img_[k]) vdo_frame_images_destroy(img_[k]);
  if (tr_sta_) vdo_tracks_destroy(tr_sta_);
  if (tr_dyn_) vdo_tracks_destroy(tr_dyn_);
  if (lm_cam_) vdo_flow2_batch_destroy(lm_cam_);
  if (lm_obj_) vdo_flow2_batch_destroy(lm_obj_);
}

int FramePipeline::ReserveObjectSlots(int n_objects, int max_points) {
  if (n_objects <= obj_slots_ && max_points <= obj_cap_) return 0;
  const int slots = std::max(obj_slots_, (n_objects + 3) / 4 * 4), cap = std::max(obj_cap_, (max_points + 2047) / 2048 * 2048);
  std::vector<int32_t> ocap(slots, cap);
  vdo_flow2_batch* nb = nullptr;
  VDO_TRY(vdo_flow2_batch_reserve(ctx_obj_, slots, ocap.data(), &nb));
  if (lm_obj_) vdo_flow2_batch_destroy(lm_obj_);
  lm_obj_ = nb; obj_slots_ = slots; obj_cap_ = cap;
  return 0;
}

int FramePipeline::PackLm(vdo_flow2_batch* b, int slot, const std::vector<int32_t>& sub, const StaSet& S, ObjBuf& B, const double* T0, double info_prior, int max_it) {
  B.ob.clear(); B.fl.clear(); B.dp.clear();
  for (int id : sub) { B.ob.push_back(S.x[id]); B.ob.push_back(S.y[id]); B.fl.push_back(S.fx[id]); B.fl.push_back(S.fy[id]); B.dp.push_back(S.d[id]); }
  vdo_flow2_problem p;
  std::memset(&p, 0, sizeof p);
  p.n = (int)sub.size(); p.obs = B.ob.data(); p.flow = B.fl.data(); p.depth = B.dp.data();
  for (int i = 0; i < 4; ++i) p.K[i] = p_.K4[i];
  float Twl[16];
  inv_rigid(Tcw_last_, Twl);
  for (int i = 0; i < 16; ++i) { p.Twl[i] = Twl[i]; p.T0[i] = T0[i]; }
  p.info_flow = 0.1; p.info_prior = info_prior; p.huber_delta = (double)std::sqrt(0.04f); p.chi2_gate = (double)0.04f;
  p.max_iterations = max_it; p.ref_quirks = 1;
  return vdo_flow2_batch_set(b, slot, &p);
}

int FramePipeline::SeedRansac(vdo_flow2_batch* b, int slot, const double* T, float* init) {
  double T0[16];
  for (int i = 0; i < 16; ++i) T0[i] = (double)(float)T[i];
  VDO_TRY(vdo_flow2_batch_set_T0(b, slot, T0));
  if (init) for (int i = 0; i < 16; ++i) init[i] = (float)T0[i];
  return 0;
}

int FramePipeline::CameraStage() {
  SecTimer t{ms_};
  cam_run_ = nullptr; cam_n_pts_ = 0; cam_n_ransac_ = 0; cam_n_mm_ = 0;
  const int n_s = have_last_ ? (int)sta_.cx.size() : 0;
  if (have_last_ && n_s >= 4) {
    std::vector<double>&X = cam_X_, &uvd = cam_uvd_;
    X.resize(3 * (size_t)n_s); uvd.resize(2 * (size_t)n_s);
    for (int i = 0; i < n_s; ++i) {
      X[3 * i] = sta_.xyz[3 * i]; X[3 * i + 1] = sta_.xyz[3 * i + 1]; X[3 * i + 2] = sta_.xyz[3 * i + 2];
      uvd[2 * i] = sta_.cx[i]; uvd[2 * i + 1] = sta_.cy[i];
// ... 1 lines not shown
    vdo_pnp_problem pp{n_s, X.data(), uvd.data(), {p_.K4[0], p_.K4[1], p_.K4[2], p_.K4[3]}, 500, 0.4, 0.98, p_.pnp_refit};
    vdo_pnp_result pr;
    inl_ransac_cam_.assign(n_s, 0);
    float MM[16];
    int32_t mm = 0;
    bool use_ransac = false;
    int rc_set = VDO_OK;
    std::function<void()> count_mm = [&] {
      mul44(vel_, Tcw_last_, MM);
      inl_mm_cam_.resize(n_s);
      mm = count_mm_inliers(MM, p_.K4, n_s, nullptr, sta_.xyz.data(), sta_.cx.data(), sta_.cy.data(), inl_mm_cam_.data());
    };
    std::function<void()> pack_lm = [&] {
      if (!lm_cam_) return;
      use_ransac = pr.n_inliers > mm;
      const std::vector<uint8_t>& flag = use_ransac ? inl_ransac_cam_ : inl_mm_cam_;
      double T0[16];
      for (int i = 0; i < 16; ++i) T0[i] = (double)MM[i];
      cam_subset_.clear();
      for (int i = 0; i < n_s; ++i) if (flag[i]) cam_subset_.push_back(i);
      rc_set = PackLm(lm_cam_, 0, cam_subset_, sta_, cam_buf_, T0, 0.3, 100);
      cam_run_ = lm_cam_; cam_n_pts_ = (int)cam_subset_.size();
      for (int i = 0; i < 16; ++i) Tcw_init_[i] = (float)T0[i];
    };
    auto call = [](void* f) { (*static_cast<std::function<void()>*>(f))(); };
    uint8_t* rip = inl_ransac_cam_.data();
    VDO_TRY(vdo_pnp_ransac_batch_gated(ctx_, 1, &pp, &pr, &rip, &mm, +call, &count_mm, +call, &pack_lm));
    cam_n_ransac_ = pr.n_inliers; cam_n_mm_ = mm;
    if (rc_set != VDO_OK) { std::fprintf(stderr, "FramePipeline: %s\n", vdo_last_error()); return -1; }
    if (lm_cam_ && use_ransac && SeedRansac(lm_cam_, 0, pr.T, Tcw_init_) != 0) return -1;
  } else if (lm_cam_) {
    for (int i = 0; i < 16; ++i) Tcw_init_[i] = Tcw_last_[i];
    VDO_TRY(vdo_flow2_batch_set(lm_cam_, 0, nullptr));
    if (have_last_) { cam_run_ = lm_cam_; cam_n_pts_ = 0; }
  }
  if (cam_run_) VDO_TRY(vdo_flow2_batch_run(cam_run_));
  t.tick(kSecK1K11RansacCam);
  return 0;
}

int FramePipeline::Step(const uint8_t* d_gray, const float* d_depth_raw, const float* d_flow, const int32_t* d_mask,
                        vdo_flow2_batch* cam, vdo_flow2_batch* obj, int n_cam_pts, int n_obj_problems, FrameCounts* out) {
  if (!ok_) return -1;
  const auto t_step0 = std::chrono::steady_clock::now();
  ev_on_ = sw_.events; ev_t0_ = t_step0;
  double ms0[kSecCount];
  for (int i = 0; i < kSecCount; ++i) ms0[i] = ms_[i];
  orb_ready_.store(0, std::memory_order_relaxed); objects_done_.store(0, std::memory_order_relaxed); mask_final_.store(0, std::memory_order_relaxed);
  StepState s(*this, d_gray, d_depth_raw, d_flow, d_mask, cam, obj, n_cam_pts, n_obj_problems);
  if (StartOrb(s) != 0) return -1;
  if (pending_ && worker_) {
    vdo_frame_images_set_ctx(ho_.img, ctx_w_);
    worker_->run([this, sp = &s] { return FinishObjects(&sp->fc, true); });
    s.fin_async = true;
  }
  if (IngestImages(s) != 0) return -1;
  if (CameraAndLateUpload(s) != 0) return -1;
  if (sw_.chain_split && have_last_ && !pending_ && BeginChain(s) != 0) return -1;
  mark(kEvChainBegun);
  if (ConsumeCamera(s) != 0) return -1;
  if (JoinLastObjects(s) != 0) return -1;
  if (EndChain(s) != 0) return -1;
  if (s.tail_async && !s.tail_on_orb && worker_->wait() != 0) return -1;
  if (have_last_ && worker_) {
    vdo_frame_images_set_ctx(s.cur, ctx_w_);
    worker_->run([this, sp = &s] { return StaticStage(*sp); });
    s.static_async = true;
  }
  if (!have_last_) { if (InitFirstFrame(s) != 0) return -1; }
  else {
    if (ObjectProblems(s) != 0) return -1;
    if (s.obj) VDO_TRY(vdo_flow2_batch_run(s.obj));
    mark(kEvObjLmLaunched);
    if (s.static_async) {
      const int rc = worker_->wait();
      vdo_frame_images_set_ctx(s.cur, ctx_);
      if (rc != 0) return -1;
    } else if (StaticStage(s) != 0) return -1;
    if ((s.tail_on_orb || s.k10_via_orb) && worker_orb_->wait() != 0) return -1;
    if (s.k10_via_orb) s.fc.n_object_samples = s.n_tmp;
    if (s.k9_via_orb) s.fc.n_static_new = s.n_new_s;
    mark(kEvStaticJoined);
    s.t.reset();
    ho_.n_objects = s.n_objects; ho_.obj_run = s.obj; ho_.n_obj_problems = s.n_obj_problems; ho_.n_tmp = s.n_tmp; ho_.img = s.cur; ho_.f_id = f_id_; ho_.tmp_idx = cur_;
    std::memcpy(ho_.Tcw, s.Tcw, sizeof s.Tcw);
    pending_ = true;
  }
  s.t.tick(kSecTracklets);
  CommitFrame(s);
  if (sw_.cam_ahead && lm_cam_ && !cam_ahead_) {
    if (CameraStage() != 0) return -1;
    cam_ahead_ = true;
    mark(kEvCamStageDone);
  }
  if (host_inputs_ && depth_inout_ && !depth_metric_ && pending_ && !p_.defer_objects) {
    VDO_TRY(vdo_frame_images_download_depth(img_[cur_ ^ 1], depth_inout_));
    depth_on_host_ = true;
  }
  if (pending_ && !p_.defer_objects) { if (FinishObjects(&s.fc) != 0) return -1; mark(kEvObjDone); }
  mark(kEvStepEnd);
  if (sw_.trace_slow) {
    const double tot = std::chrono::duration<double, std::milli>(std::chrono::steady_clock::now() - t_step0).count();
    if (tot > 2.5) {
      std::fprintf(stderr, "[slow step f=%d] %.2f ms:", f_id_ - 1, tot);
      for (int i = 0; i < kSecCount; ++i) std::fprintf(stderr, " [%d] %.2f", i, ms_[i] - ms0[i]);
      std::fprintf(stderr, "\n");
    }
  }
  if (out) *out = s.fc;
  return 0;
}

int FramePipeline::StartOrb(StepState& s) {
  s.orb_pending = worker_orb_ && !p_.use_sample_feature;
  s.tail_via_orb = s.orb_pending && pending_ && worker_;
  s.k10_via_orb = s.orb_pending && have_last_ && worker_;
  s.k9_via_orb = s.k10_via_orb && !sw_.k9_in_static;
  if (s.orb_pending) {
    worker_orb_->run([this, sp = &s] { return OrbJob(*sp); });
    s.orb_started = true;
  } else if (orb_split_ && !p_.use_sample_feature) VDO_TRY(vdo_orb_extract_begin(orb_, s.d_gray, p_.width, host_inputs_ ? 0 : 1));
  return 0;
}

int FramePipeline::OrbJob(StepState& s) {
  SecTimer t{ms_};
  int rc = vdo_orb_extract(orb_, s.d_gray, p_.width, host_inputs_ ? 0 : 1, &s.kp) == VDO_OK ? 0 : -1;
  t.tick(kSecOrb);
  if (rc != 0) std::fprintf(stderr, "FramePipeline: %s\n", vdo_last_error());
  mark(kEvOrbDone);
  orb_ready_.store(rc == 0 ? s.tag : -s.tag, std::memory_order_release);
  if (s.tail_via_orb && await_tag(objects_done_, s.tag) == s.tag) {
    const int rc2 = FinishObjectsTail(&s.fc);
    tail_done_.store(true, std::memory_order_release);
    if (rc2 != 0) rc = rc2;
  }
  if (s.k10_via_orb && await_tag(mask_final_, s.tag) == s.tag && (s.k9_via_orb && rc == 0 ? FiltersOnOrb(s) : SampleObjectsOnOrb(s)) != 0) rc = -1;
  return rc;
}

void FramePipeline::SizeFilterOutputs(int n) {
  keep_.resize(std::max(n, 1));
  for (auto* v : {&flt_cx_, &flt_cy_, &flt_fx_, &flt_fy_, &flt_d_}) v->resize(std::max(n, 1));
}
void FramePipeline::SizeSampleOutputs(ObjSet& tmp) {
  const int cap_s = SampleCap();
  tmp.x.resize(cap_s); tmp.y.resize(cap_s); tmp.cx.resize(cap_s); tmp.cy.resize(cap_s); tmp.fx.resize(cap_s); tmp.fy.resize(cap_s); tmp.d.resize(cap_s); tmp.sem.resize(cap_s);
}

int FramePipeline::SampleObjectsOnOrb(StepState& s) {
  SecTimer t{ms_};
  ObjSet& tmp = s.tmp;
  SizeSampleOutputs(tmp);
  VDO_TRY(vdo_frame_object_sample_on(ctx_orb_, s.cur, p_.th_depth_obj, 4, SampleCap(), tmp.x.data(), tmp.y.data(), tmp.cx.data(), tmp.cy.data(), tmp.fx.data(), tmp.fy.data(), tmp.d.data(),
                                     tmp.sem.data(), &s.n_tmp));
  t.tick(kSecK10OnOrb);
  return 0;
}

int FramePipeline::FiltersOnOrb(StepState& s) {
  SecTimer t{ms_};
  ObjSet& tmp = s.tmp;
  SizeFilterOutputs(s.kp.n);
  SizeSampleOutputs(tmp);
  VDO_TRY(vdo_frame_filters_on(ctx_orb_, s.cur, s.kp.n, kx_.data(), ky_.data(), p_.th_depth_bg, 0, keep_.data(), flt_cx_.data(), flt_cy_.data(), flt_fx_.data(), flt_fy_.data(),
                               flt_d_.data(), &s.n_new_s, p_.th_depth_obj, 4, SampleCap(), tmp.x.data(), tmp.y.data(), tmp.cx.data(), tmp.cy.data(), tmp.fx.data(), tmp.fy.data(),
// ... 260 lines not shown
}

int FramePipeline::ObjectProblems(StepState& s) {
  const int n_o = s.n_o;
  vdo_dyn_obj_params dp{p_.width, p_.height, 25, 50, p_.sf_mg_thres, p_.sf_ds_thres, p_.th_depth_obj, f_id_};
  std::vector<int32_t>&off = ho_.off, &idx = ho_.idx, &osem = ho_.osem, &omod = ho_.omod;
  off.assign(n_o + 2, 0); idx.resize(std::max(n_o, 1)); osem.resize(n_o + 1); omod.resize(n_o + 1);
  int n_objects = 0;
  VDO_TRY(vdo_dyn_obj_tracking(&dp, n_o, obj_sem_.data(), ho_.olab.data(), obj_.cx.data(), obj_.cy.data(), obj_depth_.data(), flow3d_.data(), obj_.sem.data(),
                               (int)last_sem_pos_.size(), last_sem_pos_.data(), last_mod_label_.data(), last_obj_stat_.data(), &max_id_,
                               off.data(), idx.data(), osem.data(), omod.data(), &n_objects));
  s.fc.n_objects = s.n_objects = n_objects;
  s.t.tick(kSecK13DynObj); mark(kEvDynObj);
  if (n_objects > 0) {
    std::vector<double>&X = obj_X_, &uvd = obj_uvd_;
    X.resize(3 * (size_t)off[n_objects] + 3); uvd.resize(2 * (size_t)off[n_objects] + 2);
    std::vector<vdo_pnp_problem> pp(n_objects);
    std::vector<vdo_pnp_result> pr(n_objects);
    for (int a = 0; a < n_objects; ++a) {
      for (int q = off[a]; q < off[a + 1]; ++q) {
        const int id = idx[q];
        X[3 * q] = obj_.xyz[3 * id]; X[3 * q + 1] = obj_.xyz[3 * id + 1]; X[3 * q + 2] = obj_.xyz[3 * id + 2];
        uvd[2 * q] = obj_.cx[id]; uvd[2 * q + 1] = obj_.cy[id];
      }
      pp[a] = vdo_pnp_problem{off[a + 1] - off[a], X.data() + 3 * (size_t)off[a], uvd.data() + 2 * (size_t)off[a], {p_.K4[0], p_.K4[1], p_.K4[2], p_.K4[3]}, 500, 0.4, 0.98, p_.pnp_refit};
    }
    inl_ransac_.assign((size_t)off[n_objects] + 1, 0);
    std::vector<uint8_t*> rip(n_objects);
    for (int a = 0; a < n_objects; ++a) rip[a] = inl_ransac_.data() + off[a];
    inl_mm_.assign((size_t)off[n_objects] + 1, 0);
    ho_.use_mm.assign(n_objects, 0);
    obj_mm_.resize(16 * (size_t)n_objects);
    std::vector<int> mm_cnt(n_objects, -1);
    int rc_pack = 0;
    std::function<void()> count_mm = [&] { CountObjectMotionModels(s.Tcw, n_objects, mm_cnt.data()); };
    std::function<void()> pack_lms = [&] { rc_pack = PackObjectLms(n_objects, pr.data(), mm_cnt.data()); };
    auto call = [](void* f) { (*static_cast<std::function<void()>*>(f))(); };
    if (sw_.mm_overlap) VDO_TRY(vdo_pnp_ransac_batch_gated(ctx_, n_objects, pp.data(), pr.data(), rip.data(), mm_cnt.data(), +call, &count_mm, +call, &pack_lms));
    else { VDO_TRY(vdo_pnp_ransac_batch(ctx_, n_objects, pp.data(), pr.data(), rip.data())); count_mm(); pack_lms(); }
    if (rc_pack != 0) { if (rc_pack == -2) std::fprintf(stderr, "FramePipeline: %s\n", vdo_last_error()); return -1; }
    for (int a = 0; a < n_objects; ++a) s.fc.n_ransac_obj += pr[a].n_inliers;
    for (int a = 0; a < n_objects; ++a) {
      if (mm_cnt[a] < 0) continue;
      s.fc.n_mm_inliers_obj += mm_cnt[a];
      if (ho_.use_mm[a]) ++s.fc.n_motion_model_obj;
    }
    if (lm_obj_) {
      for (int a = 0; a < n_objects; ++a) if (ho_.stat[a] && !ho_.use_mm[a] && SeedRansac(lm_obj_, a, pr[a].T, nullptr) != 0) return -1;
      s.obj = lm_obj_; s.n_obj_problems = obj_slots_;
    }
  } else if (lm_obj_) {
    for (int a = 0; a < obj_slots_; ++a) VDO_TRY(vdo_flow2_batch_set(lm_obj_, a, nullptr));
    s.obj = nullptr;
  }
  s.t.tick(kSecRansacObj); mark(kEvObjLmBuilt);
  return 0;
}

void FramePipeline::CommitFrame(StepState& s) {
  StaSet& nsta = s.nsta; ObjSet& nobj = s.nobj;
  const float* Tcw = s.Tcw;
  s.fc.n_static_tracked = (int)nsta.x.size();
  int64_t np = 0;
  vdo_tracks_size(tr_sta_, &s.fc.n_static_tracks, &np);
  if (keep_graph_) {
    store_.sta.append(nsta.x.size(), nsta.x.data(), nsta.y.data(), nsta.d.data(), nsta.xyz.data());
    float Twc_m[16];
    inv_rigid(Tcw, Twc_m);
    store_.add_camera(Twc_m);
    if (!have_last_) store_.dyn.append(nobj.x.size(), nobj.x.data(), nobj.y.data(), nobj.d.data(), nobj.xyz.data());
  }
  sta_ = std::move(nsta);
  if (!have_last_) { s.fc.n_object_tracked = (int)nobj.x.size(); obj_ = std::move(nobj); vdo_tracks_size(tr_dyn_, &s.fc.n_dynamic_tracks, &np); }
  float Twl[16];
  inv_rigid(Tcw_last_, Twl);
  mul44(Tcw, Twl, vel_);
  inv_rigid(vel_, cam_motion_);
  std::memcpy(Tcw_last_, Tcw, sizeof s.Tcw);
  std::memcpy(Tcw_out_, Tcw, sizeof s.Tcw);
  cur_ ^= 1; have_last_ = true; ++f_id_;
  gate_last_ = gate_cur_;
}

int FramePipeline::FinishObjects(FrameCounts* fcp, bool defer_tail) {
  if (!pending_) return 0;
  FrameCounts dummy{};
  FrameCounts& fc = fcp ? *fcp : dummy;
  SecTimer t{ms_};
  const int n_objects = ho_.n_objects, n_tmp = ho_.n_tmp, n_obj_problems = ho_.n_obj_problems;
  vdo_flow2_batch* obj = ho_.obj_run;
  const float* Tcw = ho_.Tcw;
  std::vector<int32_t>&olab = ho_.olab, &off = ho_.off, &idx = ho_.idx, &osem = ho_.osem, &omod = ho_.omod;
  ObjSet& tmp = tmpb_[ho_.tmp_idx];
  ObjSet nobj;
  std::vector<int32_t> dyn_asso;
  float Twc[16];
  inv_rigid(Tcw, Twc);
  motions_.clear();
  {
    cur_ox_ = obj_.cx; cur_oy_ = obj_.cy;
    std::vector<uint8_t> stat(std::max(n_objects, 1), 1);
    std::vector<int32_t>*p_off = &off, *p_idx = &idx;
    if (obj && obj == lm_obj_) {
      const int NS = n_obj_problems;
      std::vector<vdo_flow2_result>& rs = lm_rs_;
      std::vector<std::vector<double>>& fo = lm_fo_; std::vector<std::vector<uint8_t>>& io = lm_io_;
      std::vector<double*>& fop = lm_fop_; std::vector<uint8_t*>& iop = lm_iop_;
      rs.resize(NS); fop.resize(NS); iop.resize(NS);
      if ((int)fo.size() < NS) { fo.resize(NS); io.resize(NS); }
      for (int a = 0; a < NS; ++a) {
        const size_t na = (a < n_objects && ho_.stat[a]) ? ho_.subsets[a].size() : 0;
        fo[a].resize(2 * na + 2); io[a].resize(na + 1);
        fop[a] = fo[a].data(); iop[a] = io[a].data();
      }
      VDO_TRY(vdo_flow2_batch_fetch(obj, rs.data(), fop.data(), iop.data()));
      mark(kEvObjLmFetched);
      if (sw_.trace_obj) {
        std::fprintf(stderr, "[obj lm f=%d]", ho_.f_id);
        for (int a = 0; a < n_objects; ++a)
          if (ho_.stat[a]) std::fprintf(stderr, " sem %d n %zu its %d trials %d inl %d |", osem[a], ho_.subsets[a].size(), rs[a].iterations, rs[a].trials, rs[a].n_inliers);
        std::fprintf(stderr, "\n");
      }
      inl_off_.assign(1, 0); inl_idx_.clear();
      for (int a = 0; a < n_objects; ++a) {
        stat[a] = ho_.stat[a];
        if (stat[a]) {
          const std::vector<int32_t>& sub = ho_.subsets[a];
          for (size_t j = 0; j < sub.size(); ++j) {
            if (!io[a][j]) { olab[sub[j]] = -1; continue; }
            inl_idx_.push_back(sub[j]);
            cur_ox_[sub[j]] = key_plus_flow(obj_.x[sub[j]], fo[a][2 * j]); cur_oy_[sub[j]] = key_plus_flow(obj_.y[sub[j]], fo[a][2 * j + 1]);
          }
          ObjectMotion om; om.mod_label = omod[a]; om.sem_label = osem[a]; om.n_inliers = rs[a].n_inliers;
          float TH[16];
          for (int i = 0; i < 16; ++i) TH[i] = (float)rs[a].T[i];
          mul44(Twc, TH, om.H);
          motions_.push_back(om);
        } else {
          for (int q = off[a]; q < off[a + 1]; ++q) inl_idx_.push_back(idx[q]);
        }
        inl_off_.push_back((int32_t)inl_idx_.size());
      }
      if (inl_idx_.empty()) inl_idx_.push_back(0);
      p_off = &inl_off_; p_idx = &inl_idx_;
    } else if (obj) {
      std::vector<vdo_flow2_result> rs(std::max(n_obj_problems, 1));
      VDO_TRY(vdo_flow2_batch_fetch(obj, rs.data(), nullptr, nullptr));
    }
    t.tick(kSecWaitObjLm);
    const int cap_o = (*p_off)[n_objects] + n_tmp + 8;
    nobj.x.resize(cap_o); nobj.y.resize(cap_o); nobj.cx.resize(cap_o); nobj.cy.resize(cap_o); nobj.fx.resize(cap_o); nobj.fy.resize(cap_o); nobj.d.resize(cap_o);
    nobj.sem.resize(cap_o); nobj.label.resize(cap_o); dyn_asso.resize(cap_o);
    int mo = 0;
    nobj.xyz.resize(3 * (size_t)std::max(cap_o, 1));
    VDO_TRY(vdo_renew_object_world(ho_.img, n_objects, p_off->data(), p_idx->data(), stat.data(), osem.data(), omod.data(), cur_ox_.data(), cur_oy_.data(), olab.data(),
                                   n_tmp, tmp.x.data(), tmp.y.data(), tmp.d.data(), tmp.sem.data(), tmp.fx.data(), tmp.fy.data(), tmp.cx.data(), tmp.cy.data(),
                                   p_.max_track_obj, cap_o, p_.K4, Twc, nobj.x.data(), nobj.y.data(), nobj.d.data(), nobj.sem.data(), nobj.fx.data(), nobj.fy.data(),
                                   nobj.cx.data(), nobj.cy.data(), dyn_asso.data(), nobj.label.data(), nobj.xyz.data(), &mo));
    for (auto* v : {&nobj.x, &nobj.y, &nobj.cx, &nobj.cy, &nobj.fx, &nobj.fy, &nobj.d}) v->resize(mo);
    nobj.sem.resize(mo); nobj.label.resize(mo); dyn_asso.resize(mo);
    nobj.xyz.resize(3 * (size_t)std::max(mo, 1));
    t.tick(kSecRenewObject); mark(kEvObjRenewed);
    last_sem_pos_.assign(osem.begin(), osem.begin() + n_objects);
    last_mod_label_.assign(omod.begin(), omod.begin() + n_objects);
    last_obj_stat_.assign(stat.begin(), stat.begin() + n_objects);
    last_obj_mod_.assign(16 * (size_t)n_objects, 0.f);
    for (int a = 0, m = 0; a < n_objects; ++a) {
      float* Hd = last_obj_mod_.data() + 16 * (size_t)a;
      if (obj && obj == lm_obj_ && stat[a] && m < (int)motions_.size()) std::memcpy(Hd, motions_[m++].H, 64);
      else std::memcpy(Hd, kI4, 64);
    }
  }
  fc.n_object_tracked = (int)nobj.x.size();
  obj_ = std::move(nobj);
  if (!p_.defer_objects && !obj_.cx.empty())
    VDO_TRY(vdo_object_chain_prestage(ctx_, (int)obj_.cx.size(), obj_.sem.data(), obj_.cx.data(), obj_.cy.data(), obj_.x.data(), obj_.y.data(), obj_.d.data()));
  ho_.dyn_asso_tail = std::move(dyn_asso);
  ho_.tail_has_lm = obj && obj == lm_obj_;
  pending_ = false; tail_pending_ = true;
  return defer_tail ? 0 : FinishObjectsTail(&fc);
}

int FramePipeline::FinishObjectsTail(FrameCounts* fcp) {
  if (!tail_pending_) return 0;
  FrameCounts dummy{};
  FrameCounts& fc = fcp ? *fcp : dummy;
  SecTimer t{ms_};
  const ObjSet& nobj = obj_;
  const int f_id_obj = ho_.f_id;
  VDO_TRY(vdo_tracks_add_frame(tr_dyn_, (int)nobj.x.size(), ho_.dyn_asso_tail.data(), nobj.label.data()));
  t.tick(kSecTracklets);
  int64_t np = 0;
  vdo_tracks_size(tr_dyn_, &fc.n_dynamic_tracks, &np);
  if (keep_graph_) {
    store_.dyn.append(nobj.x.size(), nobj.x.data(), nobj.y.data(), nobj.d.data(), nobj.xyz.data());
    std::vector<float> mots(cam_motion_, cam_motion_ + 16); std::vector<int32_t> labs(1, 0);
    if (ho_.tail_has_lm)
      for (const ObjectMotion& om : motions_) { mots.insert(mots.end(), om.H, om.H + 16); labs.push_back(om.mod_label); }
    store_.add_motions((int)labs.size(), mots.data(), labs.data());
    const int Wn = p_.window_size, Ov = p_.overlap_size;
    if (Wn > 0 && Wn > Ov && (f_id_obj - Ov + 1) % (Wn - Ov) == 0 && f_id_obj >= Wn - 1 && store_.sta.frames() == f_id_obj + 1) {
      const auto t_gt0 = std::chrono::steady_clock::now();
      if (GetTracks(&tl_sta_, nullptr, f_id_obj + 1 - Wn) != 0) return -1;
      if (sw_.trace_batch) std::fprintf(stderr, "[partial batch] static tracklets flattened in %.2f ms (%zu tracks, %zu entries)\n", std::chrono::duration<double, std::milli>(std::chrono::steady_clock::now() - t_gt0).count(), tl_sta_.off.size() - 1, tl_sta_.frame.size());
      try { Optimizer::PartialBatchOptimization(store_, tl_sta_, p_.K4, Wn); }
      catch (const std::exception& e) { std::fprintf(stderr, "FramePipeline: %s\n", e.what()); return -1; }
      ++n_partial_batches_;
    }
  }
  tail_pending_ = false;
  return 0;
}

int FramePipeline::StepHost(const uint8_t* gray, const float* depth, const float* flow, const int32_t* mask, bool depth_is_metric, FrameCounts* out, float* depth_inout) {
  host_inputs_ = true; depth_metric_ = depth_is_metric; depth_inout_ = depth_inout;
  const int rc = Step(gray, depth, flow, mask, nullptr, nullptr, 0, 0, out);
  host_inputs_ = false; depth_metric_ = false; depth_inout_ = nullptr;
  return rc;
}

int FramePipeline::StepDevice(const uint8_t* d_gray, const float* d_depth, const float* d_flow, const int32_t* d_mask, bool depth_is_metric, FrameCounts* out) {
  depth_metric_ = depth_is_metric;
  const int rc = Step(d_gray, d_depth, d_flow, d_mask, nullptr, nullptr, 0, 0, out);
  depth_metric_ = false;
  return rc;
}

int FramePipeline::DownloadMask(int32_t* mask_out) {
  VDO_TRY(vdo_frame_images_download_mask(img_[cur_ ^ 1], mask_out));
  return 0;
}

int FramePipeline::DownloadDepth(float* depth_out) {
  VDO_TRY(vdo_frame_images_download_depth(img_[cur_ ^ 1], depth_out));
  return 0;
}

int FramePipeline::FinalizeMap() {
  if (!map_) return -1;
  if (pending_ && FinishObjects(nullptr) != 0) return -1;
  return SyncMap();
// ... 149 lines not shown
```

vdo_slam_amd/host/FramePipeline.h:

```cpp
#pragma once
#include <chrono>
#include <cstdint>
#include <functional>
#include <memory>
#include <atomic>
#include <vector>

#include "../../include/vdo_slam_hip.h"
#include "GraphStore.h"
#include "Map.h"

namespace VDO_SLAM {

struct PipelineParams {
  int width, height;
  float K4[4];
  float bf, depth_map_factor;
  float th_depth_bg, th_depth_obj;
  int max_track_bg, max_track_obj;
  float sf_mg_thres, sf_ds_thres;
  int n_features, n_levels, ini_th, min_th; float scale_factor;
  int build_lm;
  int defer_objects;
  int use_sample_feature;
  int sample_seed;
  int pnp_refit;
  int window_size, overlap_size;
};

struct FrameCounts { int n_orb, n_static_new, n_object_samples, n_static_tracked, n_object_tracked, n_objects, n_recovered_masks, n_static_tracks, n_dynamic_tracks,
                         n_ransac_cam, n_motion_model_cam, n_ransac_obj, n_cam_inliers, cam_lm_iterations,
                         n_mm_inliers_obj,
                         n_motion_model_obj; };

class FramePipeline {
 public:
  FramePipeline(vdo_ctx* ctx, vdo_ctx* ctx_lm, const PipelineParams& p, vdo_ctx* ctx_obj = nullptr, vdo_ctx* ctx_worker = nullptr, vdo_ctx* ctx_orb = nullptr);
  ~FramePipeline();
  int Step(const uint8_t* d_gray, const float* d_depth_raw, const float* d_flow, const int32_t* d_mask,
           vdo_flow2_batch* cam, vdo_flow2_batch* obj, int n_cam_pts, int n_obj_problems, FrameCounts* out);
  int StepHost(const uint8_t* gray, const float* depth, const float* flow, const int32_t* mask, bool depth_is_metric, FrameCounts* out, float* depth_inout = nullptr);
  int StepDevice(const uint8_t* d_gray, const float* d_depth, const float* d_flow, const int32_t* d_mask, bool depth_is_metric, FrameCounts* out);
  bool DepthConvertedOnHost() const { return depth_on_host_; }
  void SetObjectGate(const int* labels, int n) { gate_on_ = true; gate_cur_.assign(labels, labels + n); }
  int DownloadMask(int32_t* mask_out);
  int DownloadDepth(float* depth_out);
  vdo_frame_images* LastImages() { return img_[cur_ ^ 1]; }
  void KeepGraph() { keep_graph_ = true; }
  void AttachMap(Map* m) { map_ = m; keep_graph_ = true; }
  int SyncMap();
  int FinalizeMap();
  int FullBatchOptimization();
  const GraphStore& store() const { return store_; }
  int n_partial_batches_ = 0;
  int Flush(FrameCounts* fc = nullptr) { return FinishObjects(fc); }
  int GetTracks(TrackList* sta, TrackList* dyn, int first_frame = -1);
  bool ok() const { return ok_; }
  void SetDeferObjects(bool on) { p_.defer_objects = on ? 1 : 0; }
  const PipelineParams& params() const { return p_; }
  struct ObjectMotion { int mod_label, sem_label, n_inliers; float H[16]; };
  std::vector<ObjectMotion> motions_;
  float Tcw_out_[16] = {1, 0, 0, 0, 0, 1, 0, 0, 0, 0, 1, 0, 0, 0, 0, 1};
  enum { kSecK1K11RansacCam = 0, kSecOrb, kSecK9K10, kSecWaitCamLm, kSecK13DynObj, kSecRenewStatic, kSecWaitObjLm, kSecRenewObject, kSecTracklets, kSecRansacObj,
         kSecK15K11Objects, kSecK10OnOrb, kSecCount };
  double ms_[kSecCount] = {0};
  enum { kEvInputs = 0, kEvCamFetched, kEvObjChain, kEvDynObj, kEvObjLmBuilt, kEvObjLmLaunched, kEvOrbDevice, kEvOrbDone, kEvFilters, kEvStaticDone,
         kEvStaticJoined, kEvCamStageDone, kEvObjLmFetched, kEvObjRenewed, kEvObjDone, kEvStepEnd, kEvChainBegun, kEvCount };
  double ev_ms_[kEvCount] = {0}; long ev_n_[kEvCount] = {0};
  bool ev_on_ = false;
  std::chrono::steady_clock::time_point ev_t0_;
  void mark(int k) { if (ev_on_) { ev_ms_[k] += std::chrono::duration<double, std::milli>(std::chrono::steady_clock::now() - ev_t0_).count(); ++ev_n_[k]; } }

  struct StaSet { std::vector<float> x, y, cx, cy, fx, fy, d, xyz; };
  struct ObjSet : StaSet { std::vector<int32_t> sem, label; };
  const StaSet& StaticSet() const { return sta_; }
  const ObjSet& ObjectSet() const { return obj_; }
  const ObjSet& ObjectSamples() const { return tmpb_[ho_.tmp_idx]; }
  int NumObjectSamples() const { return ho_.n_tmp; }
  const std::vector<int32_t>& ObjSemPosition() const { return last_sem_pos_; }
  const std::vector<int32_t>& ObjModLabel() const { return last_mod_label_; }
  const std::vector<uint8_t>& ObjStat() const { return last_obj_stat_; }
  const std::vector<float>& ObjMod() const { return last_obj_mod_; }
  int MaxId() const { return max_id_; }

 private:
  struct Switches { bool events, trace_slow, trace_obj, trace_batch, sync_upload, async_upload, chain_split, fused_static, k9_in_static, mm_overlap, cam_ahead; };
  static Switches ReadSwitches();
  const Switches sw_ = ReadSwitches();
  struct StepState;
  int StartOrb(StepState& s), OrbJob(StepState& s), SampleObjectsOnOrb(StepState& s), FiltersOnOrb(StepState& s), JoinOrb(StepState& s);
  int IngestImages(StepState& s);
  int CameraAndLateUpload(StepState& s);
  int BeginChain(StepState& s);
  int ConsumeCamera(StepState& s);
  int JoinLastObjects(StepState& s);
  int EndChain(StepState& s);
  int FrameFilters(StepState& s), StaticStage(StepState& s);
  int InitFirstFrame(StepState& s);
  int ObjectProblems(StepState& s);
  void CommitFrame(StepState& s);
  int CameraStage();
  int FinishObjects(FrameCounts* fc, bool defer_tail = false);
  int FinishObjectsTail(FrameCounts* fc);
  void CountObjectMotionModels(const float* Tcw, int n_objects, int* cnt);
  int PackObjectLms(int n_objects, const vdo_pnp_result* pr, const int* mm_cnt);
  int SampleCap() const { return ((p_.width + 3) / 4) * ((p_.height + 3) / 4); }
  void SizeFilterOutputs(int n);
  void SizeSampleOutputs(ObjSet& tmp);
  bool tail_pending_ = false;
  GraphStore store_;
  TrackList tl_sta_, tl_dyn_;
  bool keep_graph_ = false;
  bool host_inputs_ = false, depth_metric_ = false, gate_on_ = false;
  float* depth_inout_ = nullptr;
  bool depth_on_host_ = false;
  std::vector<int> gate_cur_, gate_last_;
  Map* map_ = nullptr;
  float cam_motion_[16];
  class Worker;
  std::unique_ptr<Worker> worker_;
  std::unique_ptr<Worker> worker_orb_;
  std::atomic<bool> tail_done_{true};
  bool orb_split_ = false;
  vdo_ctx *ctx_, *ctx_lm_, *ctx_obj_, *ctx_w_, *ctx_orb_ = nullptr;
  struct ObjHandOver {
    std::vector<int32_t> olab, off, idx, osem, omod;
    int n_objects = 0, n_obj_problems = 0, n_tmp = 0, f_id = 0, tmp_idx = 0;
    vdo_flow2_batch* obj_run = nullptr; vdo_frame_images* img = nullptr; float Tcw[16];
    std::vector<std::vector<int32_t>> subsets;
    std::vector<uint8_t> stat, use_mm;
    std::vector<int32_t> dyn_asso_tail; bool tail_has_lm = false;
  } ho_;
  bool pending_ = false;
  PipelineParams p_;
  vdo_orb* orb_ = nullptr;
  vdo_frame_images* img_[2] = {nullptr, nullptr};
  vdo_tracks *tr_sta_ = nullptr, *tr_dyn_ = nullptr;
  int cur_ = 0, f_id_ = 0;
  bool ok_ = false, have_last_ = false;
  int32_t max_id_ = 1;
  StaSet sta_;
  ObjSet tmpb_[2];
  std::atomic<int> orb_ready_{0};
  std::atomic<int> objects_done_{0};
  std::atomic<int> mask_final_{0};
  ObjSet obj_;
  std::vector<int32_t> last_sem_pos_, last_mod_label_; std::vector<uint8_t> last_obj_stat_;
  std::vector<float> last_obj_mod_;
  float Tcw_last_[16], vel_[16];
  std::vector<float> kx_, ky_, kr_, ka_, ks_; std::vector<int32_t> ko_;
  std::vector<float> stat_depth_, obj_depth_, flow3d_;
  std::vector<int32_t> obj_sem_, keep_, tm_;
  std::vector<float> flt_cx_, flt_cy_, flt_fx_, flt_fy_, flt_d_;
  std::vector<float> cur_sx_, cur_sy_, cur_ox_, cur_oy_, src_x_, src_y_;
  std::vector<double> flow_out_; std::vector<uint8_t> inl_out_, inl_ransac_;
  std::vector<double> obj_X_, obj_uvd_, cam_X_, cam_uvd_;
  int obj_slots_ = 8, obj_cap_ = 6000;
  int ReserveObjectSlots(int n_objects, int max_points);
  struct ObjBuf { std::vector<double> ob, fl, dp; };
  int PackLm(vdo_flow2_batch* b, int slot, const std::vector<int32_t>& sub, const StaSet& S, ObjBuf& B, const double* T0, double info_prior, int max_it);
  int SeedRansac(vdo_flow2_batch* b, int slot, const double* T, float* init);
  vdo_flow2_batch *lm_cam_ = nullptr, *lm_obj_ = nullptr;
  std::vector<int32_t> cam_subset_, inl_off_, inl_idx_;
  std::vector<vdo_flow2_result> lm_rs_; std::vector<std::vector<double>> lm_fo_; std::vector<std::vector<uint8_t>> lm_io_;
  std::vector<double*> lm_fop_; std::vector<uint8_t*> lm_iop_;
  std::vector<uint8_t> inl_mm_;
  std::vector<float> obj_mm_;
  std::vector<ObjBuf> obj_buf_; ObjBuf cam_buf_;
  float Tcw_init_[16];
  bool cam_ahead_ = false;
  vdo_flow2_batch* cam_run_ = nullptr;
  int cam_n_pts_ = 0, cam_n_ransac_ = 0, cam_n_mm_ = 0;
  std::vector<uint8_t> inl_ransac_cam_, inl_mm_cam_;
};

}
```

vdo_slam_amd/tracking.py:

```python
import ctypes as C

import numpy as np

from . import _capi as K


def _f(a): return np.ascontiguousarray(a, dtype=np.float32)
def _i(a): return np.ascontiguousarray(a, dtype=np.int32)
def _fp(a): return a.ctypes.data_as(K.c_float_p)
def _ip(a): return a.ctypes.data_as(K.c_int32_p)


_bound = False


def _lib():
    global _bound
    L = K.lib()
    if not _bound:
        fp, ip, vp = K.c_float_p, K.c_int32_p, C.c_void_p
        L.vdo_propagate_static.argtypes = [vp, C.c_int, fp, fp, fp]
        L.vdo_propagate_object.argtypes = [vp, C.c_int, fp, fp, C.c_float, fp, ip]
        L.vdo_get3d_world.argtypes = [vp, C.c_int, fp, fp, fp, fp, fp, fp]
        L.vdo_scene_flow.argtypes = [vp, C.c_int, fp, fp, fp, ip, fp, fp, fp, fp, ip, fp, fp, fp, ip]
# ... 86 lines not shown
    if world is not None:
        out["xyz"] = xyz[:n]
    return k9, out


def mask_at(images, cx, cy):
    cx, cy = _f(cx), _f(cy)
    out = np.zeros(cx.size, np.int32)
    K.check(_lib().vdo_mask_at(images._h, cx.size, _fp(cx), _fp(cy), _ip(out)))
    return out


def mask_warp(cur_images, last_images, label):
    K.check(_lib().vdo_mask_warp(cur_images._h, last_images._h, int(label)))


class DynObjParamsC(C.Structure):
    _fields_ = [("img_w", C.c_int32), ("img_h", C.c_int32), ("shrink_row", C.c_int32), ("shrink_col", C.c_int32),
                ("sf_mg_thres", C.c_float), ("sf_ds_thres", C.c_float), ("th_depth_obj", C.c_float), ("f_id", C.c_int32)]


def _u8p(a): return a.ctypes.data_as(K.c_uint8_p)


def dyn_obj_tracking(prm: DynObjParamsC, sem_label, obj_label, key_x, key_y, depth, flow3d, last_sem_label,
                     last_sem_pos, last_mod_label, last_obj_stat, max_id):
    sem, ol = _i(sem_label), _i(obj_label).copy()
    kx, ky, d, fl, ls = _f(key_x), _f(key_y), _f(depth), _f(flow3d), _i(last_sem_label)
    lsp, lml = _i(last_sem_pos), _i(last_mod_label)
    lst = np.ascontiguousarray(last_obj_stat, dtype=np.uint8)
    n = sem.size
    nl = max(1, np.unique(sem).size)
    off = np.zeros(nl + 1, np.int32); idx = np.zeros(max(n, 1), np.int32); osem = np.zeros(nl, np.int32); omod = np.zeros(nl, np.int32)
    mid = C.c_int32(max_id); nobj = C.c_int()
    L = K.lib()
    L.vdo_dyn_obj_tracking.argtypes = [C.POINTER(DynObjParamsC), C.c_int, K.c_int32_p, K.c_int32_p, K.c_float_p, K.c_float_p, K.c_float_p, K.c_float_p,
                                       K.c_int32_p, C.c_int, K.c_int32_p, K.c_int32_p, K.c_uint8_p, C.POINTER(C.c_int32),
                                       K.c_int32_p, K.c_int32_p, K.c_int32_p, K.c_int32_p, C.POINTER(C.c_int)]
    K.check(L.vdo_dyn_obj_tracking(C.byref(prm), n, _ip(sem), _ip(ol), _fp(kx), _fp(ky), _fp(d), _fp(fl), _ip(ls), lsp.size, _ip(lsp), _ip(lml), _u8p(lst),
                                   C.byref(mid), _ip(off), _ip(idx), _ip(osem), _ip(omod), C.byref(nobj)))
    k = nobj.value
    return dict(obj_label=ol, objects=[idx[off[a]:off[a + 1]].copy() for a in range(k)], sem=osem[:k].copy(), mod=omod[:k].copy(), max_id=mid.value)


def renew_object(images, inl_sets, obj_stat, sem_pos, mod_label, cur_x, cur_y, cur_obj_label, tmp, max_num_obj, cap=None, world=None):
    off = np.zeros(len(inl_sets) + 1, np.int32)
    off[1:] = np.cumsum([len(s) for s in inl_sets])
    idx = _i(np.concatenate([np.asarray(s, np.int32) for s in inl_sets])) if len(inl_sets) and off[-1] else np.zeros(1, np.int32)
    st = np.ascontiguousarray(obj_stat, dtype=np.uint8)
    sp, ml = _i(sem_pos), _i(mod_label)
    cx, cy, col = _f(cur_x), _f(cur_y), _i(cur_obj_label)
    t = {k: (_i(v) if k == "label" else _f(v)) for k, v in tmp.items()}
    n_tmp = t["x"].size
    cap = cap or (int(off[-1]) + n_tmp + 8)
    f = [np.zeros(cap, np.float32) for _ in range(7)]
    sem = np.zeros(cap, np.int32); inl = np.zeros(cap, np.int32); ol = np.zeros(cap, np.int32)
    n = C.c_int()
    L = K.lib()
    fp, ip = K.c_float_p, K.c_int32_p
    L.vdo_renew_object.argtypes = [C.c_void_p, C.c_int, ip, ip, K.c_uint8_p, ip, ip, fp, fp, ip, C.c_int, fp, fp, fp, ip, fp, fp, fp, fp, C.c_int, C.c_int,
                                   fp, fp, fp, ip, fp, fp, fp, fp, ip, ip, C.POINTER(C.c_int)]
    if world is None:
        K.check(L.vdo_renew_object(images._h, len(inl_sets), _ip(off), _ip(idx), _u8p(st), _ip(sp), _ip(ml), _fp(cx), _fp(cy), _ip(col),
                                   n_tmp, _fp(t["x"]), _fp(t["y"]), _fp(t["depth"]), _ip(t["label"]), _fp(t["flow_x"]), _fp(t["flow_y"]), _fp(t["corr_x"]), _fp(t["corr_y"]),
                                   max_num_obj, cap, _fp(f[0]), _fp(f[1]), _fp(f[2]), _ip(sem), _fp(f[3]), _fp(f[4]), _fp(f[5]), _fp(f[6]), _ip(inl), _ip(ol), C.byref(n)))
    else:
        K4, Twc = _f(world[0]), _f(world[1])
        xyz = np.zeros((cap, 3), np.float32)
        L.vdo_renew_object_world.argtypes = [C.c_void_p, C.c_int, ip, ip, K.c_uint8_p, ip, ip, fp, fp, ip, C.c_int, fp, fp, fp, ip, fp, fp, fp, fp, C.c_int, C.c_int, fp, fp,
                                             fp, fp, fp, ip, fp, fp, fp, fp, ip, ip, fp, C.POINTER(C.c_int)]
        K.check(L.vdo_renew_object_world(images._h, len(inl_sets), _ip(off), _ip(idx), _u8p(st), _ip(sp), _ip(ml), _fp(cx), _fp(cy), _ip(col),
                                         n_tmp, _fp(t["x"]), _fp(t["y"]), _fp(t["depth"]), _ip(t["label"]), _fp(t["flow_x"]), _fp(t["flow_y"]), _fp(t["corr_x"]), _fp(t["corr_y"]),
                                         max_num_obj, cap, _fp(K4), _fp(Twc), _fp(f[0]), _fp(f[1]), _fp(f[2]), _ip(sem), _fp(f[3]), _fp(f[4]), _fp(f[5]), _fp(f[6]), _ip(inl), _ip(ol),
                                         _fp(xyz), C.byref(n)))
    m = n.value
    names = ("key_x", "key_y", "depth", "flow_x", "flow_y", "corr_x", "corr_y")
    out = {k: a[:m] for k, a in zip(names, f)}
    out.update(sem=sem[:m], inlier_id=inl[:m], obj_label=ol[:m])
    if world is not None:
        out["xyz"] = xyz[:m]
    return out


def update_mask(cur_images, last_images, last_sem_label, last_corr_x, last_corr_y):
    sl, cx, cy = _i(last_sem_label), _f(last_corr_x), _f(last_corr_y)
    n = C.c_int()
    L = K.lib()
    L.vdo_update_mask.argtypes = [C.c_void_p, C.c_void_p, C.c_int, K.c_int32_p, K.c_float_p, K.c_float_p, C.POINTER(C.c_int)]
    K.check(L.vdo_update_mask(cur_images._h, last_images._h, sl.size, _ip(sl), _fp(cx), _fp(cy), C.byref(n)))
    return n.value


def object_chain(cur_images, last_images, last_sem_label, last_corr_x, last_corr_y, th_depth_obj, Tcw_cur, last_x, last_y, last_d, Tcw_last, K4):
    sl, cx, cy = _i(last_sem_label), _f(last_corr_x), _f(last_corr_y)
    lx, ly, ld = _f(last_x), _f(last_y), _f(last_d)
    Tc, Tl, K4 = _f(Tcw_cur), _f(Tcw_last), _f(K4)
    n = sl.size
    rec = C.c_int()
    d = np.zeros(n, np.float32); sem = np.zeros(n, np.int32); fl = np.zeros((n, 3), np.float32); ol = np.zeros(n, np.int32)
    L = K.lib()
    L.vdo_object_chain.argtypes = [C.c_void_p, C.c_void_p, C.c_int, K.c_int32_p, K.c_float_p, K.c_float_p, C.c_float, K.c_float_p, K.c_float_p, K.c_float_p, K.c_float_p,
                                   K.c_float_p, K.c_float_p, C.POINTER(C.c_int), K.c_float_p, K.c_int32_p, K.c_float_p, K.c_int32_p]
    K.check(L.vdo_object_chain(cur_images._h, last_images._h, n, _ip(sl), _fp(cx), _fp(cy), th_depth_obj, _fp(Tc), _fp(lx), _fp(ly), _fp(ld), _fp(Tl), _fp(K4),
                               C.byref(rec), _fp(d), _ip(sem), _fp(fl), _ip(ol)))
    return rec.value, d, sem, fl, ol


class ObjectChain:

    def __init__(self, cur_images, last_images, last_sem_label, last_corr_x, last_corr_y, last_x, last_y, last_d):
        self._cur = cur_images
        self._in = (_i(last_sem_label), _f(last_corr_x), _f(last_corr_y), _f(last_x), _f(last_y), _f(last_d))
        sl, cx, cy, lx, ly, ld = self._in
        L = K.lib()
        L.vdo_object_chain_begin.argtypes = [C.c_void_p, C.c_void_p, C.c_int, K.c_int32_p] + [K.c_float_p] * 5
        K.check(L.vdo_object_chain_begin(cur_images._h, last_images._h, sl.size, _ip(sl), _fp(cx), _fp(cy), _fp(lx), _fp(ly), _fp(ld)))

    def end(self, th_depth_obj, Tcw_cur, Tcw_last, K4):
        Tc, Tl, K4 = _f(Tcw_cur), _f(Tcw_last), _f(K4)
        n = self._in[0].size
        rec = C.c_int()
        d = np.zeros(n, np.float32); sem = np.zeros(n, np.int32); fl = np.zeros((n, 3), np.float32); ol = np.zeros(n, np.int32)
        L = K.lib()
        L.vdo_object_chain_end.argtypes = [C.c_void_p, C.c_float, K.c_float_p, K.c_float_p, K.c_float_p, C.POINTER(C.c_int), K.c_float_p, K.c_int32_p, K.c_float_p, K.c_int32_p]
        K.check(L.vdo_object_chain_end(self._cur._h, th_depth_obj, _fp(Tc), _fp(Tl), _fp(K4), C.byref(rec), _fp(d), _ip(sem), _fp(fl), _ip(ol)))
        return rec.value, d, sem, fl, ol


def object_chain_prestage(ctx, last_sem_label, last_corr_x, last_corr_y, last_x, last_y, last_d):
    sl, cx, cy = _i(last_sem_label), _f(last_corr_x), _f(last_corr_y)
    lx, ly, ld = _f(last_x), _f(last_y), _f(last_d)
    L = K.lib()
    L.vdo_object_chain_prestage.argtypes = [C.c_void_p, C.c_int, K.c_int32_p, K.c_float_p, K.c_float_p, K.c_float_p, K.c_float_p, K.c_float_p]
    K.check(L.vdo_object_chain_prestage(ctx._h, sl.size, _ip(sl), _fp(cx), _fp(cy), _fp(lx), _fp(ly), _fp(ld)))


class TrackBuilder:

    def __init__(self, with_object_label=False):
        L = K.lib()
        L.vdo_tracks_create.argtypes = [C.c_int, C.POINTER(C.c_void_p)]
        L.vdo_tracks_destroy.argtypes = [C.c_void_p]
        L.vdo_tracks_add_frame.argtypes = [C.c_void_p, C.c_int, K.c_int32_p, K.c_int32_p]
        L.vdo_tracks_size.argtypes = [C.c_void_p, C.POINTER(C.c_int), C.POINTER(C.c_int64)]
        L.vdo_tracks_get.argtypes = [C.c_void_p, K.c_int32_p, K.c_int32_p, K.c_int32_p, K.c_int32_p]
        self.with_label = with_object_label
        self._h = C.c_void_p()
        K.check(L.vdo_tracks_create(int(with_object_label), C.byref(self._h)))

    def add_frame(self, asso, feat_label=None):
        a = _i(asso)
        lab = _i(feat_label) if feat_label is not None else None
        K.check(K.lib().vdo_tracks_add_frame(self._h, a.size, _ip(a), _ip(lab) if lab is not None else None))

    def get(self):
        nt, npairs = C.c_int(), C.c_int64()
        K.check(K.lib().vdo_tracks_size(self._h, C.byref(nt), C.byref(npairs)))
        off = np.zeros(nt.value + 1, np.int32); fr = np.zeros(max(npairs.value, 1), np.int32); ft = np.zeros(max(npairs.value, 1), np.int32)
        oid = np.zeros(max(nt.value, 1), np.int32)
        K.check(K.lib().vdo_tracks_get(self._h, _ip(off), _ip(fr), _ip(ft), _ip(oid)))
        return off, fr[:npairs.value], ft[:npairs.value], (oid[:nt.value] if self.with_label else None)

    def close(self):
        if self._h:
            K.lib().vdo_tracks_destroy(self._h); self._h = C.c_void_p()

# ... 10 lines not shown
```

Measured before the change: 1544.

## Queue object renewal on device directly from flow2 LM outputs

Adds a queue/collect API so object renewal kernels read flow2 LM flow and inlier outputs directly from device memory and are enqueued behind the LM kernel. The host no longer syncs and fetches LM results before launching renewal, which removes a host round trip and lets the renewal be collected in one wait. A pipeline switch selects the queued path, and the added state in the context and batch raises lifetime and ordering complexity.

```diff
diff --git a/include/vdo_slam_hip.h b/include/vdo_slam_hip.h
--- a/include/vdo_slam_hip.h
+++ b/include/vdo_slam_hip.h
@@ -137,6 +137,7 @@
 int vdo_flow2_batch_set_T0(vdo_flow2_batch* batch, int k, const double T0[16]);
 int vdo_flow2_batch_run(vdo_flow2_batch* batch);
 int vdo_flow2_batch_fetch(vdo_flow2_batch* batch, vdo_flow2_result* results, double** flow_out, uint8_t** inlier_out);
+int vdo_flow2_batch_device_outputs(vdo_flow2_batch* batch, vdo_ctx** ctx, const double** d_flow, const uint8_t** d_inlier, int32_t* slot_off, int* n_problems);
 int vdo_flow2_batch_destroy(vdo_flow2_batch* batch);
 int vdo_flow2_optimize(vdo_ctx* ctx, const vdo_flow2_problem* p, vdo_flow2_result* result, double* flow_out, uint8_t* inlier_out);
 
@@ -331,6 +332,18 @@
                            int max_num_obj, int cap, const float K4[4], const float Twc[16],
                            float* key_x, float* key_y, float* depth_out, int32_t* sem_out, float* flow_x, float* flow_y,
                            float* corr_x, float* corr_y, int32_t* dyn_inlier_id, int32_t* obj_label_out, float* xyz_out, int* n_out);
+int vdo_renew_object_world_queue(vdo_flow2_batch* batch, vdo_frame_images* f, int n_obj, const uint8_t* obj_stat, const int32_t* slot_off, const int32_t* slot_idx,
+                                 int n_keys, const float* key_x, const float* key_y,
+                                 int n_tmp, const float* tmp_x, const float* tmp_y, const float* tmp_depth, const float K4[4], const float Twc[16]);
+int vdo_renew_object_world_collect(vdo_flow2_batch* batch, vdo_flow2_result* results, double** flow_out, uint8_t** inlier_out,
+                                   void (*after_wait)(void*), void* after_wait_arg,
+                                   const int32_t* sem_pos, const int32_t* mod_label, const int32_t* cur_obj_label,
+                                   const float* tmp_x, const float* tmp_y, const float* tmp_depth, const int32_t* tmp_label,
+                                   const float* tmp_flow_x, const float* tmp_flow_y, const float* tmp_corr_x, const float* tmp_corr_y,
+                                   int max_num_obj, int cap,
+                                   float* key_x, float* key_y, float* depth_out, int32_t* sem_out, float* flow_x, float* flow_y,
+                                   float* corr_x, float* corr_y, int32_t* dyn_inlier_id, int32_t* obj_label_out, float* xyz_out, int* n_out,
+                                   float* cand_x, float* cand_y);
 
 int vdo_update_mask(vdo_frame_images* cur, vdo_frame_images* last, int n, const int32_t* last_sem_label,
                     const float* last_corr_x, const float* last_corr_y, int* n_recovered);
diff --git a/vdo_slam_amd/csrc/capi_ctx.hip b/vdo_slam_amd/csrc/capi_ctx.hip
--- a/vdo_slam_amd/csrc/capi_ctx.hip
+++ b/vdo_slam_amd/csrc/capi_ctx.hip
@@ -55,6 +55,10 @@
     hipStreamSynchronize(ctx->stream);
     ctx->chain_open_free(ctx->chain_open);
   }
+  if (ctx->renew_open) {
+    hipStreamSynchronize(ctx->stream);
+    ctx->renew_open_free(ctx->renew_open);
+  }
   if (ctx->d_arena) hipFree(ctx->d_arena);
   if (ctx->h_arena) hipHostFree(ctx->h_arena);
   if (ctx->ba_slab) hipFree(ctx->ba_slab);
diff --git a/vdo_slam_amd/csrc/ctx.hpp b/vdo_slam_amd/csrc/ctx.hpp
--- a/vdo_slam_amd/csrc/ctx.hpp
+++ b/vdo_slam_amd/csrc/ctx.hpp
@@ -12,6 +12,7 @@
   char* h_arena = nullptr; size_t h_cap = 0;
   char* h_arena_dev = nullptr;
   void* chain_open = nullptr; void (*chain_open_free)(void*) = nullptr; bool arena_held = false;
+  void* renew_open = nullptr; void (*renew_open_free)(void*) = nullptr; void* renew_open_batch = nullptr;
   char* d_stage = nullptr; char* h_stage = nullptr; size_t stage_cap = 0;
   int stage_n = -1, stage_L = 0;
   int32_t stage_uni[64]; int32_t stage_off[65];
diff --git a/vdo_slam_amd/csrc/flow2.hip b/vdo_slam_amd/csrc/flow2.hip
--- a/vdo_slam_amd/csrc/flow2.hip
+++ b/vdo_slam_amd/csrc/flow2.hip
@@ -7,6 +7,7 @@
 
 #include "../../include/vdo_slam_hip.h"
 #include "ctx.hpp"
+#include "flow2_shared.hpp"
 #include "lm_dev.hpp"
 
 namespace vdo {
@@ -600,11 +601,16 @@
   bool probs_dirty = false;
   unsigned run_seq = 0;
   const Flow2Dev* d_probs_run = nullptr;
+  bool out_valid = false;
 };
 
 extern "C" int vdo_flow2_batch_destroy(vdo_flow2_batch* b) {
   if (!b) return VDO_OK;
   if (b->ctx) { ctx_bind(b->ctx); hipStreamSynchronize(b->ctx->stream); }
+  if (b->ctx && b->ctx->renew_open && b->ctx->renew_open_batch == b) {
+    b->ctx->renew_open_free(b->ctx->renew_open);
+    b->ctx->renew_open = nullptr; b->ctx->renew_open_batch = nullptr; b->ctx->arena_held = false;
+  }
   for (void* p : b->allocs) hipFree(p);
   if (b->h_pin) hipHostFree(b->h_pin);
   if (b->h_up) hipHostFree(b->h_up);
@@ -722,6 +728,7 @@
   }
   d.n = n; b->ns[k] = n;
   b->probs_dirty = true;
+  b->out_valid = false;
   return VDO_OK;
 }
 
@@ -759,6 +766,22 @@
   hipLaunchKernelGGL(k_flow2_lm, dim3(((b->n_problems + 7) / 8) * 8 * F2_CLUSTER), dim3(F2_THREADS), 0, b->ctx->stream, b->d_probs_run ? b->d_probs_run : (const Flow2Dev*)b->d_probs, b->A);
   hipError_t e = hipGetLastError();
   if (e != hipSuccess) return set_error(VDO_ERR_NO_DEVICE, "k_flow2_lm launch: %s", hipGetErrorString(e));
+  b->out_valid = true;
+  return VDO_OK;
+}
+
+extern "C" int vdo_flow2_batch_device_outputs(vdo_flow2_batch* b, vdo_ctx** ctx, const double** d_flow, const uint8_t** d_inlier, int32_t* slot_off, int* n_problems) {
+  if (!b) return set_error(VDO_ERR_INVALID, "vdo_flow2_batch_device_outputs: null handle");
+  if (!b->h_up) return set_error(VDO_ERR_INVALID, "vdo_flow2_batch_device_outputs: batch not created by vdo_flow2_batch_reserve");
+  if (!b->out_valid) return set_error(VDO_ERR_INVALID, "vdo_flow2_batch_device_outputs: no vdo_flow2_batch_run since the last vdo_flow2_batch_set");
+  size_t used = 0;
+  for (int k = 0; k < b->n_problems; ++k) { if (slot_off) slot_off[k] = (int32_t)used; used += (size_t)b->ns[k]; }
+  if (slot_off) slot_off[b->n_problems] = (int32_t)used;
+  const double* pf = (const double*)(b->A.out + sizeof(vdo_flow2_result) * (size_t)b->n_problems);
+  if (ctx) *ctx = b->ctx;
+  if (d_flow) *d_flow = pf;
+  if (d_inlier) *d_inlier = (const uint8_t*)(pf + 2 * used);
+  if (n_problems) *n_problems = b->n_problems;
   return VDO_OK;
 }
 
@@ -766,11 +789,17 @@
   if (!b || !results) return set_error(VDO_ERR_INVALID, "null argument");
   int rc = ctx_bind(b->ctx);
   if (rc != VDO_OK) return rc;
+  hipError_t e = hipStreamSynchronize(b->ctx->stream);
+  if (e != hipSuccess) return set_error(VDO_ERR_NO_DEVICE, "flow2 fetch: %s", hipGetErrorString(e));
+  return flow2_batch_unpack(b, results, flow_out, inlier_out);
+}
+
+vdo_ctx* vdo::flow2_batch_ctx(vdo_flow2_batch* b) { return b->ctx; }
+
+int vdo::flow2_batch_unpack(vdo_flow2_batch* b, vdo_flow2_result* results, double** flow_out, uint8_t** inlier_out) {
   const size_t NP = (size_t)b->n_problems;
   size_t used = 0;
   for (int k = 0; k < b->n_problems; ++k) used += (size_t)b->ns[k];
-  hipError_t e = hipStreamSynchronize(b->ctx->stream);
-  if (e != hipSuccess) return set_error(VDO_ERR_NO_DEVICE, "flow2 fetch: %s", hipGetErrorString(e));
   const vdo_flow2_result* pr = (const vdo_flow2_result*)b->h_pin;
   const double* pf = (const double*)(b->h_pin + sizeof(vdo_flow2_result) * NP);
   const uint8_t* pi = (const uint8_t*)(pf + 2 * used);
diff --git a/vdo_slam_amd/csrc/flow2_shared.hpp b/vdo_slam_amd/csrc/flow2_shared.hpp
--- /dev/null
+++ b/vdo_slam_amd/csrc/flow2_shared.hpp
@@ -0,0 +1,7 @@
+#pragma once
+#include "../../include/vdo_slam_hip.h"
+
+namespace vdo {
+vdo_ctx* flow2_batch_ctx(vdo_flow2_batch* b);
+int flow2_batch_unpack(vdo_flow2_batch* b, vdo_flow2_result* results, double** flow_out, uint8_t** inlier_out);
+}
diff --git a/vdo_slam_amd/csrc/tracking_logic.hip b/vdo_slam_amd/csrc/tracking_logic.hip
--- a/vdo_slam_amd/csrc/tracking_logic.hip
+++ b/vdo_slam_amd/csrc/tracking_logic.hip
@@ -10,6 +10,7 @@
 #include "near_flags.hpp"
 #include "arena.hpp"
 #include "tracking_shared.hpp"
+#include "flow2_shared.hpp"
 
 namespace vdo {
 
@@ -37,7 +38,7 @@
                                 int32_t* __restrict__ ok, int32_t* __restrict__ sem, float* __restrict__ dout, float* __restrict__ fx, float* __restrict__ fy,
                                 Cam cam, float* __restrict__ xyz_c,
                                 int n_tmp, const float* __restrict__ qx, const float* __restrict__ qy, const float* __restrict__ qd, float* __restrict__ xyz_t,
-                                int32_t* __restrict__ used) {
+                                int32_t* __restrict__ used, const int32_t* __restrict__ valid) {
   const int i = blockIdx.x * blockDim.x + threadIdx.x;
   if (i < n) {
     const int x = (int)px[i], y = (int)py[i];
@@ -51,6 +52,7 @@
         if (x + fxe < w && y + fye < h && x + fxe > 0 && y + fye > 0) good = 1;
       }
     }
+    if (valid && !valid[i]) good = 0;
     ok[i] = good; sem[i] = sl; dout[i] = d; fx[i] = fxe; fy[i] = fye;
     float o3[3];
     backproject(cam, (float)x, (float)y, d, o3);
@@ -62,6 +64,26 @@
     backproject(cam, qx[i], qy[i], qd[i], o3);
     xyz_t[3 * i] = o3[0]; xyz_t[3 * i + 1] = o3[1]; xyz_t[3 * i + 2] = o3[2];
   }
+}
+
+__global__ void k_obj_candidates(int n, const double* __restrict__ flow, const uint8_t* __restrict__ inl, const float* __restrict__ kx, const float* __restrict__ ky,
+                                 float* __restrict__ cx, float* __restrict__ cy, float* __restrict__ hx, float* __restrict__ hy, int32_t* __restrict__ valid,
+                                 int n_tmp, const float* __restrict__ sx, const float* __restrict__ sy, const float* __restrict__ sd,
+                                 float* __restrict__ qx, float* __restrict__ qy, float* __restrict__ qd) {
+  const int i = blockIdx.x * blockDim.x + threadIdx.x;
+  if (i < n) {
+    const float x = (float)((double)kx[i] + flow[2 * (size_t)i]), y = (float)((double)ky[i] + flow[2 * (size_t)i + 1]);
+    const int fin = (x - x == 0.f && y - y == 0.f) ? 1 : 0;
+    cx[i] = x; cy[i] = y;
+    if (hx) { hx[i] = x; hy[i] = y; }
+    valid[i] = (inl[i] != 0 && fin) ? 1 : 0;
+  }
+  if (sx && i < n_tmp) { qx[i] = sx[i]; qy[i] = sy[i]; qd[i] = sd[i]; }
+}
+
+__global__ void k_words_out(int n, const int32_t* __restrict__ src, int32_t* __restrict__ dst) {
+  const int i = blockIdx.x * blockDim.x + threadIdx.x;
+  if (i < n) dst[i] = src[i];
 }
 
 constexpr int kVoteBins = 1024;
@@ -366,6 +388,15 @@
   return VDO_OK;
 }
 
+static int renew_object_select(int n_obj, const uint8_t* obj_stat, const int32_t* sem_pos, const int32_t* mod_label, const int32_t* cur_obj_label,
+                               int nc, const float* cx, const float* cy, const int32_t* cid, const int32_t* cobj, const int32_t* ok, const int32_t* sem, const float* dd,
+                               const float* fx, const float* fy, const float* xyz_c,
+                               int n_tmp, const float* tmp_x, const float* tmp_y, const float* tmp_depth, const int32_t* tmp_label,
+                               const float* tmp_flow_x, const float* tmp_flow_y, const float* tmp_corr_x, const float* tmp_corr_y, const int32_t* used, const float* xyz_t,
+                               int max_num_obj, int cap,
+                               float* key_x, float* key_y, float* depth_out, int32_t* sem_out, float* flow_x, float* flow_y,
+                               float* corr_x, float* corr_y, int32_t* dyn_inlier_id, int32_t* obj_label_out, float* xyz_out, int* n_out);
+
 extern "C" int vdo_renew_object_world(vdo_frame_images* f, int n_obj, const int32_t* inl_off, const int32_t* inl_idx, const uint8_t* obj_stat,
                                       const int32_t* sem_pos, const int32_t* mod_label,
                                       const float* cur_x, const float* cur_y, const int32_t* cur_obj_label,
@@ -404,7 +435,7 @@
       const int nmax = std::max(nc, n_tmp);
       hipLaunchKernelGGL(k_renew_obj_all, dim3((nmax + 255) / 256), dim3(256), 0, st, nc, (const float*)dx, (const float*)dy, (const int32_t*)f->d_mask,
                          (const float*)f->d_depth, (const float*)f->d_flow, f->w, f->h, dok, dsem, ddd, dfx, dfy, cam, dxc,
-                         n_tmp, (const float*)dqx, (const float*)dqy, (const float*)dqd, dxt, dused);
+                         n_tmp, (const float*)dqx, (const float*)dqy, (const float*)dqd, dxt, dused, (const int32_t*)nullptr);
       if (nc && n_tmp) launch_near_flags_sel(st, n_tmp, dqx, dqy, nc, dx, dy, dok, 1, dused, false);
     } else if (nc) {
       hipLaunchKernelGGL(k_renew_obj_pred, dim3((nc + 255) / 256), dim3(256), 0, st, nc, (const float*)dx, (const float*)dy, (const int32_t*)f->d_mask,
@@ -417,6 +448,19 @@
     rc = S.finish("vdo_renew_object");
     if (rc != VDO_OK) return rc;
   }
+  return renew_object_select(n_obj, obj_stat, sem_pos, mod_label, cur_obj_label, nc, cx.data(), cy.data(), cid.data(), cobj.data(), ok.data(), sem.data(), dd.data(),
+                             fx.data(), fy.data(), xyz_c.data(), n_tmp, tmp_x, tmp_y, tmp_depth, tmp_label, tmp_flow_x, tmp_flow_y, tmp_corr_x, tmp_corr_y, used.data(),
+                             xyz_t.data(), max_num_obj, cap, key_x, key_y, depth_out, sem_out, flow_x, flow_y, corr_x, corr_y, dyn_inlier_id, obj_label_out, xyz_out, n_out);
+}
+
+static int renew_object_select(int n_obj, const uint8_t* obj_stat, const int32_t* sem_pos, const int32_t* mod_label, const int32_t* cur_obj_label,
+                               int nc, const float* cx, const float* cy, const int32_t* cid, const int32_t* cobj, const int32_t* ok, const int32_t* sem, const float* dd,
+                               const float* fx, const float* fy, const float* xyz_c,
+                               int n_tmp, const float* tmp_x, const float* tmp_y, const float* tmp_depth, const int32_t* tmp_label,
+                               const float* tmp_flow_x, const float* tmp_flow_y, const float* tmp_corr_x, const float* tmp_corr_y, const int32_t* used, const float* xyz_t,
+                               int max_num_obj, int cap,
+                               float* key_x, float* key_y, float* depth_out, int32_t* sem_out, float* flow_x, float* flow_y,
+                               float* corr_x, float* corr_y, int32_t* dyn_inlier_id, int32_t* obj_label_out, float* xyz_out, int* n_out) {
   int m = 0;
   auto push = [&](float x, float y, float d, int sl, float flx, float fly, float crx, float cry, int inl, int ol, const float* p3) -> bool {
     if (m >= cap) return false;
@@ -431,7 +475,7 @@
   for (int k = 0; k < nc; ++k) {
     if (!ok[k]) continue;
     const int x = (int)cx[k], y = (int)cy[k];
-    if (!push((float)x, (float)y, dd[k], sem[k], fx[k], fy[k], x + fx[k], y + fy[k], cid[k], cur_obj_label[cid[k]], xyz_c.data() + 3 * (size_t)k)) return set_error(VDO_ERR_INVALID, "vdo_renew_object: output capacity %d too small", cap);
+    if (!push((float)x, (float)y, dd[k], sem[k], fx[k], fy[k], x + fx[k], y + fy[k], cid[k], cur_obj_label[cid[k]], xyz_c + 3 * (size_t)k)) return set_error(VDO_ERR_INVALID, "vdo_renew_object: output capacity %d too small", cap);
     ++fea_count[cobj[k]];
   }
   for (int i = 0; i < n_obj; ++i) {
@@ -440,7 +484,7 @@
     for (int start = 0; start < 15 && tot < max_num_obj; ++start) {
       for (int j = start; j < n_tmp; j += 15) {
         if (tmp_label[j] != sem_pos[i] || used[j]) continue;
-        if (!push(tmp_x[j], tmp_y[j], tmp_depth[j], tmp_label[j], tmp_flow_x[j], tmp_flow_y[j], tmp_corr_x[j], tmp_corr_y[j], -1, mod_label[i], xyz_t.data() + 3 * (size_t)j))
+        if (!push(tmp_x[j], tmp_y[j], tmp_depth[j], tmp_label[j], tmp_flow_x[j], tmp_flow_y[j], tmp_corr_x[j], tmp_corr_y[j], -1, mod_label[i], xyz_t + 3 * (size_t)j))
           return set_error(VDO_ERR_INVALID, "vdo_renew_object: output capacity %d too small", cap);
         if (++tot >= max_num_obj) break;
       }
@@ -457,7 +501,7 @@
   for (size_t s = 0; s < uni.size(); ++s) {
     if (known[s]) continue;
     for (int j = 0; j < n_tmp; ++j)
-      if (slot[j] == (int)s && !push(tmp_x[j], tmp_y[j], tmp_depth[j], tmp_label[j], tmp_flow_x[j], tmp_flow_y[j], tmp_corr_x[j], tmp_corr_y[j], -1, -2, xyz_t.data() + 3 * (size_t)j))
+      if (slot[j] == (int)s && !push(tmp_x[j], tmp_y[j], tmp_depth[j], tmp_label[j], tmp_flow_x[j], tmp_flow_y[j], tmp_corr_x[j], tmp_corr_y[j], -1, -2, xyz_t + 3 * (size_t)j))
         return set_error(VDO_ERR_INVALID, "vdo_renew_object: output capacity %d too small", cap);
   }
   *n_out = m;
@@ -475,6 +519,145 @@
   return vdo_renew_object_world(f, n_obj, inl_off, inl_idx, obj_stat, sem_pos, mod_label, cur_x, cur_y, cur_obj_label, n_tmp, tmp_x, tmp_y, tmp_depth, tmp_label,
                                 tmp_flow_x, tmp_flow_y, tmp_corr_x, tmp_corr_y, max_num_obj, cap, nullptr, nullptr,
                                 key_x, key_y, depth_out, sem_out, flow_x, flow_y, corr_x, corr_y, dyn_inlier_id, obj_label_out, nullptr, n_out);
+}
+
+namespace {
+struct RenewOpen {
+  Arena S;
+  int n_obj = 0, ns = 0, n_tmp = 0;
+  std::vector<uint8_t> stat;
+  std::vector<int32_t> cid, cobj;
+  const float *hx = nullptr, *hy = nullptr, *dd = nullptr, *fx = nullptr, *fy = nullptr, *xyz_c = nullptr, *xyz_t = nullptr;
+  const int32_t *ok = nullptr, *sem = nullptr, *used = nullptr;
+  explicit RenewOpen(vdo_ctx* c) : S(c) {}
+};
+void renew_open_free(void* p) { delete static_cast<RenewOpen*>(p); }
+void renew_close(vdo_ctx* ctx) {
+  if (ctx->renew_open) { renew_open_free(ctx->renew_open); ctx->renew_open = nullptr; ctx->renew_open_batch = nullptr; }
+  ctx->arena_held = false;
+}
+}
+
+extern "C" int vdo_renew_object_world_queue(vdo_flow2_batch* b, vdo_frame_images* f, int n_obj, const uint8_t* obj_stat, const int32_t* slot_off, const int32_t* slot_idx,
+                                            int n_keys, const float* key_x, const float* key_y,
+                                            int n_tmp, const float* tmp_x, const float* tmp_y, const float* tmp_depth, const float K4[4], const float Twc[16]) {
+  if (!b || !f || n_obj < 0 || n_tmp < 0 || n_keys < 0 || !K4 || !Twc || (n_obj > 0 && (!obj_stat || !slot_off)) || (n_tmp > 0 && (!tmp_x || !tmp_y || !tmp_depth)))
+    return set_error(VDO_ERR_INVALID, "vdo_renew_object_world_queue: bad argument");
+  vdo_ctx* ctx = nullptr;
+  const double* d_flow = nullptr;
+  const uint8_t* d_inl = nullptr;
+  int np = 0;
+  static thread_local std::vector<int32_t> boff;
+  int rc = vdo_flow2_batch_device_outputs(b, &ctx, nullptr, nullptr, nullptr, &np);
+  if (rc != VDO_OK) return rc;
+  boff.resize((size_t)np + 1);
+  rc = vdo_flow2_batch_device_outputs(b, &ctx, &d_flow, &d_inl, boff.data(), &np);
+  if (rc != VDO_OK) return rc;
+  if (ctx->renew_open) return set_error(VDO_ERR_INVALID, "vdo_renew_object_world_queue: a renewal is already queued on this context (collect it first)");
+  if (ctx->arena_held) return set_error(VDO_ERR_INVALID, "vdo_renew_object_world_queue: the context's scratch is held by an open object chain");
+  if (n_obj > np) return set_error(VDO_ERR_INVALID, "vdo_renew_object_world_queue: %d objects, %d slots in the batch", n_obj, np);
+  for (int a = 0; a < np; ++a) {
+    const int want = (a < n_obj && obj_stat[a]) ? slot_off[a + 1] - slot_off[a] : 0;
+    if (want < 0 || boff[a + 1] - boff[a] != want) return set_error(VDO_ERR_INVALID, "vdo_renew_object_world_queue: slot %d of the batch holds %d correspondences, the object %d", a, boff[a + 1] - boff[a], want);
+  }
+  const int ns = boff[np];
+  if (ns > 0 && (!slot_idx || !key_x || !key_y)) return set_error(VDO_ERR_INVALID, "vdo_renew_object_world_queue: bad argument");
+  rc = ctx_bind(ctx);
+  if (rc != VDO_OK) return rc;
+  RenewOpen* R = new RenewOpen(ctx);
+  R->n_obj = n_obj; R->ns = ns; R->n_tmp = n_tmp;
+  R->stat.assign(obj_stat, obj_stat + n_obj);
+  static thread_local std::vector<float> gx, gy;
+  gx.clear(); gy.clear();
+  for (int a = 0; a < n_obj; ++a) {
+    if (!obj_stat[a]) continue;
+    for (int q = slot_off[a]; q < slot_off[a + 1]; ++q) {
+      const int id = slot_idx[q];
+      if (id < 0 || id >= n_keys) { delete R; return set_error(VDO_ERR_INVALID, "vdo_renew_object_world_queue: key index %d outside [0, %d)", id, n_keys); }
+      gx.push_back(key_x[id]); gy.push_back(key_y[id]); R->cid.push_back(id); R->cobj.push_back(a);
+    }
+  }
+  Arena& S = R->S;
+  if (!S.reserve(Arena::bytes_for(24 * ((size_t)ns + (size_t)n_tmp + 64)))) { delete R; return set_error(VDO_ERR_OOM, "scratch arena: allocation failed"); }
+  const bool mapped_in = ctx->h_arena_dev && std::getenv("VDO_ARENA_NO_MAPPED_OUT") == nullptr && std::getenv("VDO_RENEW_QUEUE_COPY_IN") == nullptr;
+  auto input = [&](const float* host, size_t n) -> float* {
+    if (!mapped_in) return S.up(host, n);
+    float* d = S.out<float>(n);
+    if (d && n) std::memcpy(const_cast<float*>(S.view((const float*)d, n)), host, n * sizeof(float));
+    return d;
+  };
+  float *ikx = input(gx.data(), ns), *iky = input(gy.data(), ns);
+  float *isx = input(tmp_x, n_tmp), *isy = input(tmp_y, n_tmp), *isd = input(tmp_depth, n_tmp);
+  float *dcx = S.up<float>(nullptr, ns), *dcy = S.up<float>(nullptr, ns);
+  int32_t* dvalid = S.up<int32_t>(nullptr, ns);
+  float *dqx = isx, *dqy = isy, *dqd = isd;
+  if (mapped_in) { dqx = S.up<float>(nullptr, n_tmp); dqy = S.up<float>(nullptr, n_tmp); dqd = S.up<float>(nullptr, n_tmp); }
+  int32_t *dok = S.up<int32_t>(nullptr, ns), *dused = S.up<int32_t>(nullptr, n_tmp);
+  float *hx = S.out<float>(ns), *hy = S.out<float>(ns);
+  int32_t* dsem = S.out<int32_t>(ns);
+  float *ddd = S.out<float>(ns), *dfx = S.out<float>(ns), *dfy = S.out<float>(ns);
+  float *dxc = S.out<float>(3 * (size_t)ns), *dxt = S.out<float>(3 * (size_t)n_tmp);
+  if (!ikx || !iky || !isx || !isy || !isd || !dcx || !dcy || !dvalid || !dqx || !dqy || !dqd || !dok || !dused || !hx || !hy || !dsem || !ddd || !dfx || !dfy || !dxc || !dxt) {
+    delete R;
+    return set_error(VDO_ERR_OOM, "scratch arena: allocation failed");
+  }
+  hipStream_t st = S.stream();
+  const Cam cam = make_cam_Twc(K4, Twc);
+  const int n_gather = std::max(ns, mapped_in ? n_tmp : 0), nmax = std::max(ns, n_tmp);
+  if (n_gather)
+    hipLaunchKernelGGL(k_obj_candidates, dim3((n_gather + 255) / 256), dim3(256), 0, st, ns, d_flow, d_inl, (const float*)ikx, (const float*)iky, dcx, dcy, hx, hy, dvalid,
+                       n_tmp, mapped_in ? (const float*)isx : (const float*)nullptr, (const float*)isy, (const float*)isd, dqx, dqy, dqd);
+  if (nmax)
+    hipLaunchKernelGGL(k_renew_obj_all, dim3((nmax + 255) / 256), dim3(256), 0, st, ns, (const float*)dcx, (const float*)dcy, (const int32_t*)f->d_mask,
+                       (const float*)f->d_depth, (const float*)f->d_flow, f->w, f->h, dok, dsem, ddd, dfx, dfy, cam, dxc,
+                       n_tmp, (const float*)dqx, (const float*)dqy, (const float*)dqd, dxt, dused, (const int32_t*)dvalid);
+  if (ns && n_tmp) launch_near_flags_sel(st, n_tmp, dqx, dqy, ns, dcx, dcy, dok, 1, dused, false);
+  R->hx = S.view((const float*)hx, ns); R->hy = S.view((const float*)hy, ns);
+  R->sem = S.view((const int32_t*)dsem, ns); R->dd = S.view((const float*)ddd, ns); R->fx = S.view((const float*)dfx, ns); R->fy = S.view((const float*)dfy, ns);
+  R->xyz_c = S.view((const float*)dxc, 3 * (size_t)ns); R->xyz_t = S.view((const float*)dxt, 3 * (size_t)n_tmp);
+  if (ctx->h_arena_dev && std::getenv("VDO_RENEW_QUEUE_COPY_OUT") == nullptr) {
+    const size_t lo = (size_t)((const char*)dok - ctx->d_arena), hi = (size_t)((const char*)(dused + n_tmp) - ctx->d_arena);
+    const int words = (int)((hi - lo) / 4);
+    if (words) hipLaunchKernelGGL(k_words_out, dim3((words + 255) / 256), dim3(256), 0, st, words, (const int32_t*)(ctx->d_arena + lo), (int32_t*)(ctx->h_arena_dev + lo));
+    R->ok = (const int32_t*)(ctx->h_arena + lo); R->used = (const int32_t*)(ctx->h_arena + ((const char*)dused - ctx->d_arena));
+  } else {
+    R->ok = S.view((const int32_t*)dok, ns); R->used = S.view((const int32_t*)dused, n_tmp);
+  }
+  S.queue_downloads();
+  const hipError_t e = hipGetLastError();
+  if (e != hipSuccess) { hipStreamSynchronize(st); delete R; return set_error(VDO_ERR_NO_DEVICE, "vdo_renew_object_world_queue: %s", hipGetErrorString(e)); }
+  ctx->renew_open = R; ctx->renew_open_free = &renew_open_free; ctx->renew_open_batch = b;
+  ctx->arena_held = true;
+  return VDO_OK;
+}
+
+extern "C" int vdo_renew_object_world_collect(vdo_flow2_batch* b, vdo_flow2_result* results, double** flow_out, uint8_t** inlier_out,
+                                              void (*after_wait)(void*), void* after_wait_arg,
+                                              const int32_t* sem_pos, const int32_t* mod_label, const int32_t* cur_obj_label,
+                                              const float* tmp_x, const float* tmp_y, const float* tmp_depth, const int32_t* tmp_label,
+                                              const float* tmp_flow_x, const float* tmp_flow_y, const float* tmp_corr_x, const float* tmp_corr_y,
+                                              int max_num_obj, int cap,
+                                              float* key_x, float* key_y, float* depth_out, int32_t* sem_out, float* flow_x, float* flow_y,
+                                              float* corr_x, float* corr_y, int32_t* dyn_inlier_id, int32_t* obj_label_out, float* xyz_out, int* n_out,
+                                              float* cand_x, float* cand_y) {
+  if (!b) return set_error(VDO_ERR_INVALID, "vdo_renew_object_world_collect: null handle");
+  vdo_ctx* ctx = flow2_batch_ctx(b);
+  RenewOpen* R = static_cast<RenewOpen*>(ctx->renew_open);
+  if (!R || ctx->renew_open_batch != b) return set_error(VDO_ERR_INVALID, "vdo_renew_object_world_collect: no renewal queued behind this batch");
+  int rc = (!results || !n_out || !xyz_out || cap < 0) ? set_error(VDO_ERR_INVALID, "vdo_renew_object_world_collect: bad argument") : ctx_bind(ctx);
+  if (rc == VDO_OK) rc = R->S.finish("vdo_renew_object_world_collect");
+  else hipStreamSynchronize(ctx->stream);
+  if (after_wait) after_wait(after_wait_arg);
+  if (rc == VDO_OK) rc = flow2_batch_unpack(b, results, flow_out, inlier_out);
+  if (rc == VDO_OK) {
+    if (cand_x && R->ns) std::memcpy(cand_x, R->hx, sizeof(float) * (size_t)R->ns);
+    if (cand_y && R->ns) std::memcpy(cand_y, R->hy, sizeof(float) * (size_t)R->ns);
+    rc = renew_object_select(R->n_obj, R->stat.data(), sem_pos, mod_label, cur_obj_label, R->ns, R->hx, R->hy, R->cid.data(), R->cobj.data(), R->ok, R->sem, R->dd,
+                             R->fx, R->fy, R->xyz_c, R->n_tmp, tmp_x, tmp_y, tmp_depth, tmp_label, tmp_flow_x, tmp_flow_y, tmp_corr_x, tmp_corr_y, R->used, R->xyz_t,
+                             max_num_obj, cap, key_x, key_y, depth_out, sem_out, flow_x, flow_y, corr_x, corr_y, dyn_inlier_id, obj_label_out, xyz_out, n_out);
+  }
+  renew_close(ctx);
+  return rc;
 }
 
 extern "C" int vdo_update_mask(vdo_frame_images* cur, vdo_frame_images* last, int n, const int32_t* last_sem_label,
diff --git a/vdo_slam_amd/host/FramePipeline.cc b/vdo_slam_amd/host/FramePipeline.cc
--- a/vdo_slam_amd/host/FramePipeline.cc
+++ b/vdo_slam_amd/host/FramePipeline.cc
@@ -94,6 +94,7 @@
   w.events = on("VDO_PIPE_EVENTS"); w.trace_slow = on("VDO_PIPE_TRACE_SLOW"); w.trace_obj = on("VDO_PIPE_TRACE_OBJ"); w.trace_batch = on("VDO_BATCH_TRACE");
   w.sync_upload = on("VDO_PIPE_SYNC_UPLOAD"); w.async_upload = !on("VDO_PIPE_NO_ASYNC_UPLOAD"); w.chain_split = !on("VDO_PIPE_NO_CHAIN_SPLIT");
   w.fused_static = !on("VDO_PIPE_NO_FUSED_STATIC"); w.k9_in_static = on("VDO_PIPE_K9_IN_STATIC"); w.mm_overlap = !on("VDO_PIPE_NO_MM_OVERLAP"); w.cam_ahead = !on("VDO_PIPE_NO_CAM_AHEAD");
+  w.queued_renew = !on("VDO_PIPE_NO_QUEUED_RENEW");
   return w;
 }
 
@@ -261,6 +262,8 @@
     if (s.k9_via_orb) s.fc.n_static_new = s.n_new_s;
     mark(kEvStaticJoined);
     s.t.reset();
+    if (QueueObjectRenewal(s) != 0) return -1;
+    s.t.tick(kSecRenewObject);
     ho_.n_objects = s.n_objects; ho_.obj_run = s.obj; ho_.n_obj_problems = s.n_obj_problems; ho_.n_tmp = s.n_tmp; ho_.img = s.cur; ho_.f_id = f_id_; ho_.tmp_idx = cur_;
     std::memcpy(ho_.Tcw, s.Tcw, sizeof s.Tcw);
     pending_ = true;
@@ -687,6 +690,22 @@
   gate_last_ = gate_cur_;
 }
 
+int FramePipeline::QueueObjectRenewal(StepState& s) {
+  ho_.renew_queued = false;
+  if (!sw_.queued_renew || !s.obj || s.obj != lm_obj_ || ctx_obj_ == ctx_ || ctx_obj_ == ctx_w_ || ctx_obj_ == ctx_orb_) return 0;
+  ho_.slot_off.assign(1, 0); ho_.slot_idx.clear();
+  for (int a = 0; a < s.n_objects; ++a) {
+    if (ho_.stat[a]) ho_.slot_idx.insert(ho_.slot_idx.end(), ho_.subsets[a].begin(), ho_.subsets[a].end());
+    ho_.slot_off.push_back((int32_t)ho_.slot_idx.size());
+  }
+  float Twc[16];
+  inv_rigid(s.Tcw, Twc);
+  VDO_TRY(vdo_renew_object_world_queue(s.obj, s.cur, s.n_objects, ho_.stat.data(), ho_.slot_off.data(), ho_.slot_idx.data(), (int)obj_.x.size(), obj_.x.data(), obj_.y.data(),
+                                       s.n_tmp, s.tmp.x.data(), s.tmp.y.data(), s.tmp.d.data(), p_.K4, Twc));
+  ho_.renew_queued = true;
+  return 0;
+}
+
 int FramePipeline::FinishObjects(FrameCounts* fcp, bool defer_tail) {
   if (!pending_) return 0;
   FrameCounts dummy{};
@@ -702,8 +721,16 @@
   float Twc[16];
   inv_rigid(Tcw, Twc);
   motions_.clear();
+  auto size_outputs = [&](int cap) {
+    nobj.x.resize(cap); nobj.y.resize(cap); nobj.cx.resize(cap); nobj.cy.resize(cap); nobj.fx.resize(cap); nobj.fy.resize(cap); nobj.d.resize(cap);
+    nobj.sem.resize(cap); nobj.label.resize(cap); dyn_asso.resize(cap);
+    nobj.xyz.resize(3 * (size_t)std::max(cap, 1));
+  };
+  const bool queued = ho_.renew_queued;
+  ho_.renew_queued = false;
+  int mo = 0;
   {
-    cur_ox_ = obj_.cx; cur_oy_ = obj_.cy;
+    if (!queued) { cur_ox_ = obj_.cx; cur_oy_ = obj_.cy; }
     std::vector<uint8_t> stat(std::max(n_objects, 1), 1);
     std::vector<int32_t>*p_off = &off, *p_idx = &idx;
     if (obj && obj == lm_obj_) {
@@ -718,8 +745,19 @@
         fo[a].resize(2 * na + 2); io[a].resize(na + 1);
         fop[a] = fo[a].data(); iop[a] = io[a].data();
       }
-      VDO_TRY(vdo_flow2_batch_fetch(obj, rs.data(), fop.data(), iop.data()));
-      mark(kEvObjLmFetched);
+      if (queued) {
+        const int cap_q = (int)ho_.slot_idx.size() + n_tmp + 8;
+        size_outputs(cap_q);
+        struct AfterWait { FramePipeline* P; SecTimer* t; } aw{this, &t};
+        auto after_wait = [](void* p) { AfterWait* a = static_cast<AfterWait*>(p); a->t->tick(kSecWaitObjLm); a->P->mark(kEvObjLmFetched); };
+        VDO_TRY(vdo_renew_object_world_collect(obj, rs.data(), fop.data(), iop.data(), +after_wait, &aw, osem.data(), omod.data(), olab.data(),
+                                               tmp.x.data(), tmp.y.data(), tmp.d.data(), tmp.sem.data(), tmp.fx.data(), tmp.fy.data(), tmp.cx.data(), tmp.cy.data(),
+                                               p_.max_track_obj, cap_q, nobj.x.data(), nobj.y.data(), nobj.d.data(), nobj.sem.data(), nobj.fx.data(), nobj.fy.data(),
+                                               nobj.cx.data(), nobj.cy.data(), dyn_asso.data(), nobj.label.data(), nobj.xyz.data(), &mo, nullptr, nullptr));
+      } else {
+        VDO_TRY(vdo_flow2_batch_fetch(obj, rs.data(), fop.data(), iop.data()));
+        mark(kEvObjLmFetched);
+      }
       if (sw_.trace_obj) {
         std::fprintf(stderr, "[obj lm f=%d]", ho_.f_id);
         for (int a = 0; a < n_objects; ++a)
@@ -733,6 +771,7 @@
           const std::vector<int32_t>& sub = ho_.subsets[a];
           for (size_t j = 0; j < sub.size(); ++j) {
             if (!io[a][j]) { olab[sub[j]] = -1; continue; }
+            if (queued) continue;
             inl_idx_.push_back(sub[j]);
             cur_ox_[sub[j]] = key_plus_flow(obj_.x[sub[j]], fo[a][2 * j]); cur_oy_[sub[j]] = key_plus_flow(obj_.y[sub[j]], fo[a][2 * j + 1]);
           }
@@ -752,16 +791,15 @@
       std::vector<vdo_flow2_result> rs(std::max(n_obj_problems, 1));
       VDO_TRY(vdo_flow2_batch_fetch(obj, rs.data(), nullptr, nullptr));
     }
-    t.tick(kSecWaitObjLm);
-    const int cap_o = (*p_off)[n_objects] + n_tmp + 8;
-    nobj.x.resize(cap_o); nobj.y.resize(cap_o); nobj.cx.resize(cap_o); nobj.cy.resize(cap_o); nobj.fx.resize(cap_o); nobj.fy.resize(cap_o); nobj.d.resize(cap_o);
-    nobj.sem.resize(cap_o); nobj.label.resize(cap_o); dyn_asso.resize(cap_o);
-    int mo = 0;
-    nobj.xyz.resize(3 * (size_t)std::max(cap_o, 1));
-    VDO_TRY(vdo_renew_object_world(ho_.img, n_objects, p_off->data(), p_idx->data(), stat.data(), osem.data(), omod.data(), cur_ox_.data(), cur_oy_.data(), olab.data(),
-                                   n_tmp, tmp.x.data(), tmp.y.data(), tmp.d.data(), tmp.sem.data(), tmp.fx.data(), tmp.fy.data(), tmp.cx.data(), tmp.cy.data(),
-                                   p_.max_track_obj, cap_o, p_.K4, Twc, nobj.x.data(), nobj.y.data(), nobj.d.data(), nobj.sem.data(), nobj.fx.data(), nobj.fy.data(),
-                                   nobj.cx.data(), nobj.cy.data(), dyn_asso.data(), nobj.label.data(), nobj.xyz.data(), &mo));
+    if (!queued) {
+      t.tick(kSecWaitObjLm);
+      const int cap_o = (*p_off)[n_objects] + n_tmp + 8;
+      size_outputs(cap_o);
+      VDO_TRY(vdo_renew_object_world(ho_.img, n_objects, p_off->data(), p_idx->data(), stat.data(), osem.data(), omod.data(), cur_ox_.data(), cur_oy_.data(), olab.data(),
+                                     n_tmp, tmp.x.data(), tmp.y.data(), tmp.d.data(), tmp.sem.data(), tmp.fx.data(), tmp.fy.data(), tmp.cx.data(), tmp.cy.data(),
+                                     p_.max_track_obj, cap_o, p_.K4, Twc, nobj.x.data(), nobj.y.data(), nobj.d.data(), nobj.sem.data(), nobj.fx.data(), nobj.fy.data(),
+                                     nobj.cx.data(), nobj.cy.data(), dyn_asso.data(), nobj.label.data(), nobj.xyz.data(), &mo));
+    }
     for (auto* v : {&nobj.x, &nobj.y, &nobj.cx, &nobj.cy, &nobj.fx, &nobj.fy, &nobj.d}) v->resize(mo);
     nobj.sem.resize(mo); nobj.label.resize(mo); dyn_asso.resize(mo);
     nobj.xyz.resize(3 * (size_t)std::max(mo, 1));
diff --git a/vdo_slam_amd/host/FramePipeline.h b/vdo_slam_amd/host/FramePipeline.h
--- a/vdo_slam_amd/host/FramePipeline.h
+++ b/vdo_slam_amd/host/FramePipeline.h
@@ -84,7 +84,7 @@
   int MaxId() const { return max_id_; }
 
  private:
-  struct Switches { bool events, trace_slow, trace_obj, trace_batch, sync_upload, async_upload, chain_split, fused_static, k9_in_static, mm_overlap, cam_ahead; };
+  struct Switches { bool events, trace_slow, trace_obj, trace_batch, sync_upload, async_upload, chain_split, fused_static, k9_in_static, mm_overlap, cam_ahead, queued_renew; };
   static Switches ReadSwitches();
   const Switches sw_ = ReadSwitches();
   struct StepState;
@@ -100,6 +100,7 @@
   int ObjectProblems(StepState& s);
   void CommitFrame(StepState& s);
   int CameraStage();
+  int QueueObjectRenewal(StepState& s);
   int FinishObjects(FrameCounts* fc, bool defer_tail = false);
   int FinishObjectsTail(FrameCounts* fc);
   void CountObjectMotionModels(const float* Tcw, int n_objects, int* cnt);
@@ -130,6 +131,8 @@
     std::vector<std::vector<int32_t>> subsets;
     std::vector<uint8_t> stat, use_mm;
     std::vector<int32_t> dyn_asso_tail; bool tail_has_lm = false;
+    bool renew_queued = false;
+    std::vector<int32_t> slot_off, slot_idx;
   } ho_;
   bool pending_ = false;
   PipelineParams p_;
diff --git a/vdo_slam_amd/tracking.py b/vdo_slam_amd/tracking.py
--- a/vdo_slam_amd/tracking.py
+++ b/vdo_slam_amd/tracking.py
@@ -192,6 +192,67 @@
     return out
 
 
+def flow2_device_outputs(batch):
+    n = len(batch.problems)
+    pf, pi, ctx, npb = C.c_void_p(), C.c_void_p(), C.c_void_p(), C.c_int()
+    off = np.zeros(n + 1, np.int32)
+    L = K.lib()
+    L.vdo_flow2_batch_device_outputs.argtypes = [C.c_void_p, C.POINTER(C.c_void_p), C.POINTER(C.c_void_p), C.POINTER(C.c_void_p), K.c_int32_p, C.POINTER(C.c_int)]
+    K.check(L.vdo_flow2_batch_device_outputs(batch._h, C.byref(ctx), C.byref(pf), C.byref(pi), _ip(off), C.byref(npb)))
+    assert npb.value == n and ctx.value == batch.ctx._h.value
+    return dict(flow_ptr=pf.value, inlier_ptr=pi.value, slot_off=off)
+
+
+def renew_object_queue(batch, images, obj_stat, subsets, key_x, key_y, tmp, world):
+    off = np.zeros(len(subsets) + 1, np.int32)
+    off[1:] = np.cumsum([len(s) for s in subsets])
+    idx = _i(np.concatenate([np.asarray(s, np.int32) for s in subsets])) if len(subsets) and off[-1] else np.zeros(1, np.int32)
+    st = np.ascontiguousarray(obj_stat, dtype=np.uint8) if len(subsets) else np.zeros(1, np.uint8)
+    kx, ky = _f(key_x), _f(key_y)
+    tx, ty, td = _f(tmp["x"]), _f(tmp["y"]), _f(tmp["depth"])
+    K4, Twc = _f(world[0]), _f(world[1])
+    L = K.lib()
+    fp, ip = K.c_float_p, K.c_int32_p
+    L.vdo_renew_object_world_queue.argtypes = [C.c_void_p, C.c_void_p, C.c_int, K.c_uint8_p, ip, ip, C.c_int, fp, fp, C.c_int, fp, fp, fp, fp, fp]
+    K.check(L.vdo_renew_object_world_queue(batch._h, images._h, len(subsets), _u8p(st), _ip(off), _ip(idx), kx.size, _fp(kx), _fp(ky), tx.size, _fp(tx), _fp(ty), _fp(td),
+                                           _fp(K4), _fp(Twc)))
+    return int(sum(len(s) for a, s in enumerate(subsets) if st[a]))
+
+
+def renew_object_collect(batch, n_slots, sem_pos, mod_label, cur_obj_label, tmp, max_num_obj, cap=None):
+    n = len(batch.problems)
+    res = (K.Flow2ResultC * n)()
+    sizes = [p.n if p is not None else 0 for p in batch.problems]
+    flows = [np.zeros((m, 2)) for m in sizes]
+    inls = [np.zeros(m, np.uint8) for m in sizes]
+    flp = (K.c_double_p * n)(*[K._dp(f) for f in flows])
+    inp = (K.c_uint8_p * n)(*[a.ctypes.data_as(K.c_uint8_p) for a in inls])
+    sp, ml, col = _i(sem_pos), _i(mod_label), _i(cur_obj_label)
+    t = {k: (_i(v) if k == "label" else _f(v)) for k, v in tmp.items()}
+    n_tmp = t["x"].size
+    cap = (n_slots + n_tmp + 8) if cap is None else cap
+    f = [np.zeros(max(cap, 1), np.float32) for _ in range(7)]
+    sem = np.zeros(max(cap, 1), np.int32); inl = np.zeros(max(cap, 1), np.int32); ol = np.zeros(max(cap, 1), np.int32)
+    xyz = np.zeros((max(cap, 1), 3), np.float32)
+    candx, candy = np.zeros(max(n_slots, 1), np.float32), np.zeros(max(n_slots, 1), np.float32)
+    m = C.c_int()
+    L = K.lib()
+    fp, ip = K.c_float_p, K.c_int32_p
+    L.vdo_renew_object_world_collect.argtypes = [C.c_void_p, C.c_void_p, C.c_void_p, C.c_void_p, C.c_void_p, C.c_void_p, ip, ip, ip, fp, fp, fp, ip, fp, fp, fp, fp,
+                                                 C.c_int, C.c_int, fp, fp, fp, ip, fp, fp, fp, fp, ip, ip, fp, C.POINTER(C.c_int), fp, fp]
+    K.check(L.vdo_renew_object_world_collect(batch._h, res, flp, inp, None, None, _ip(sp), _ip(ml), _ip(col),
+                                             _fp(t["x"]), _fp(t["y"]), _fp(t["depth"]), _ip(t["label"]), _fp(t["flow_x"]), _fp(t["flow_y"]), _fp(t["corr_x"]), _fp(t["corr_y"]),
+                                             max_num_obj, cap, _fp(f[0]), _fp(f[1]), _fp(f[2]), _ip(sem), _fp(f[3]), _fp(f[4]), _fp(f[5]), _fp(f[6]), _ip(inl), _ip(ol),
+                                             _fp(xyz), C.byref(m), _fp(candx), _fp(candy)))
+    lm = [dict(T=np.array(res[i].T).reshape(4, 4), n_inliers=res[i].n_inliers, iterations=res[i].iterations, trials=res[i].trials, stop_reason=res[i].stop_reason,
+               initial_chi2=res[i].initial_chi2, final_chi2=res[i].final_chi2, final_lambda=res[i].final_lambda, flow=flows[i], inliers=inls[i]) for i in range(n)]
+    k = m.value
+    names = ("key_x", "key_y", "depth", "flow_x", "flow_y", "corr_x", "corr_y")
+    out = {q: a[:k] for q, a in zip(names, f)}
+    out.update(sem=sem[:k], inlier_id=inl[:k], obj_label=ol[:k], xyz=xyz[:k], cand_x=candx[:n_slots], cand_y=candy[:n_slots])
+    return lm, out
+
+
 def update_mask(cur_images, last_images, last_sem_label, last_corr_x, last_corr_y):
     sl, cx, cy = _i(last_sem_label), _f(last_corr_x), _f(last_corr_y)
     n = C.c_int()
```

Measured after the change: 1525. 1.3% lower.
